# renaudbedard/raytracing-in-one-weekend

Measured on AMD Instinct MI355X. Metric: Msamples/s, 486-sphere cover scene 1920x1080 8-bounce, higher is better.
Workload: dtype f32

## Files before the change

### include/rtow.h

```cpp
#ifndef RTOW_H
#define RTOW_H

#include <stddef.h>
#include <stdint.h>

#ifdef __cplusplus
extern "C" {
#endif

#if defined(_WIN32)
#define RTOW_API __declspec(dllexport)
#else
#define RTOW_API __attribute__((visibility("default")))
#endif

#define RTOW_API_VERSION 12

typedef enum RtowResult {
    RTOW_SUCCESS = 0,
    RTOW_ERROR_INVALID_VALUE = 1,
    RTOW_ERROR_MEMORY_ALLOCATION = 2,
    RTOW_ERROR_NO_DEVICE = 3,
    RTOW_ERROR_NO_SCENE = 4,
    RTOW_ERROR_UNSUPPORTED = 5,
// ... 102 lines not shown
    int32_t sceneInLds;
    uint64_t sceneBytesDevice;
    uint64_t hitSpillBytes;
    int32_t hitListCapacity;
    int32_t wideCodes;
    int32_t thresholdSet;
    int32_t schedulerTune[9];
} RtowSceneInfo;


typedef struct RtowView {
    RtowFloat3 origin;
    RtowFloat3 lowerLeftCorner;
    RtowFloat3 horizontal, vertical;
    RtowFloat3 forward, up, right;
    float lensRadius;
} RtowView;

typedef enum RtowRngPolicy { RTOW_RNG_REFERENCE = 0, RTOW_RNG_PER_SAMPLE = 1, RTOW_RNG_PER_SAMPLE_XOROSHIRO = 2 } RtowRngPolicy;

typedef enum RtowCubemapChannelType { RTOW_CUBEMAP_UNSIGNED_BYTE = 0, RTOW_CUBEMAP_SIGNED_HALF = 1 } RtowCubemapChannelType;
typedef struct RtowCubemapDesc {
    int32_t faceWidth, faceHeight;
    int32_t channelType;
    int32_t pixelStride;
    const void* faces;
} RtowCubemapDesc;

typedef struct RtowBlueNoiseDesc {
    uint32_t rowStride, textureCount;
    const void* texels;
} RtowBlueNoiseDesc;
typedef struct RtowStbNoiseDesc {
    uint32_t rowStride, textureCount;
    const void* scalar;
    const void* vector2;
    const void* cosineUnitVector3;
    const void* unitVector2;
    const void* unitVector3;
} RtowStbNoiseDesc;

typedef struct RtowEnvironment {
    int32_t skyType;
    RtowFloat3 skyBottomColor;
    RtowFloat3 skyTopColor;
} RtowEnvironment;

typedef struct RtowSampleParams {
    RtowFloat2 size;
    int32_t sliceOffset;
    int32_t sliceDivider;
    uint32_t seed;
    RtowView view;
    RtowEnvironment environment;
    uint32_t sampleCountRange[2];
    int32_t traceDepth;
    int32_t subPixelJitter;
    int32_t noiseColor;
    RtowFloat2 sampleCountWeightExtrema;
    int32_t diagnosticsStride;
    int32_t noiseTextureIndex;
    int32_t rngPolicy;
} RtowSampleParams;

typedef struct RtowAccumBuffers {
    float* color;
    float* normal;
    float* albedo;
    float* sampleCountWeight;
} RtowAccumBuffers;

typedef struct RtowContext_t* RtowContext;

typedef void (*RtowLogCallback)(int32_t level, const char* tag, const char* message, void* userData);

typedef enum RtowContextFlags {
    RTOW_CONTEXT_EXACT_TIES_ALWAYS = 1u << 0,
    RTOW_CONTEXT_EXACT_TIES_NEVER = 1u << 1,
    RTOW_CONTEXT_REFERENCE_DIAGNOSTICS = 1u << 2,
    RTOW_CONTEXT_NO_CAMERA_RAY_LISTS = 1u << 3,
    RTOW_CONTEXT_NO_CHUNK_ORDER = 1u << 4,
    RTOW_CONTEXT_FORCE_WIDE_CODES = 1u << 5,
    RTOW_CONTEXT_NO_CHAIN_FUSION = 1u << 7,
    RTOW_CONTEXT_NO_THRESHOLD_TUNING = 1u << 6
} RtowContextFlags;

typedef struct RtowContextOptions {
    int32_t deviceOrdinal;
    RtowLogCallback logCallback;
    void* logCallbackData;
    int32_t logCallbackLevel;
    uint32_t flags;
    int32_t ldsSceneBudgetBytes;
    int32_t schedulerTune[9];
    int32_t hitListCapacity;
    int32_t sliceBlockThreads;
} RtowContextOptions;

RTOW_API int rtowGetApiVersion(void);
RTOW_API const char* rtowErrorString(int result);

RTOW_API int rtowCreateContext(const RtowContextOptions* options, RtowContext* outContext);
RTOW_API int rtowDestroyContext(RtowContext context);

RTOW_API int rtowUploadScene(RtowContext context, const RtowSceneDesc* scene);
RTOW_API int rtowGetSceneInfo(RtowContext context, RtowSceneInfo* outInfo);

RTOW_API int rtowUploadSkyCubemap(RtowContext context, const RtowCubemapDesc* cubemap);

RTOW_API int rtowUploadBlueNoise(RtowContext context, const RtowBlueNoiseDesc* noise);
RTOW_API int rtowUploadStbNoise(RtowContext context, const RtowStbNoiseDesc* noise);

RTOW_API int rtowSampleBatch(RtowContext context, const RtowSampleParams* params,
                             const RtowAccumBuffers* in, const RtowAccumBuffers* out,
                             void* diagnostics, const volatile uint8_t* cancel);

RTOW_API int rtowSampleBatchDevice(RtowContext context, const RtowSampleParams* params,
                                   const RtowAccumBuffers* in, const RtowAccumBuffers* out,
                                   void* diagnostics, void* stream, const volatile uint8_t* cancel);

RTOW_API int rtowSampleBatchChainDevice(RtowContext context, int32_t count, const RtowSampleParams* params ,
                                        const RtowAccumBuffers* in, const RtowAccumBuffers* out,
                                        void* const* diagnostics , void* stream, const volatile uint8_t* cancel);

typedef struct RtowAdaptiveFeed {
    const RtowFloat2* extremaIn;
    RtowFloat2* extremaOut;
    int32_t lag;
    int32_t reserved;
} RtowAdaptiveFeed;

RTOW_API int rtowSampleBatchChainAdaptiveDevice(RtowContext context, int32_t count, const RtowSampleParams* params ,
                                                const RtowAccumBuffers* in, const RtowAccumBuffers* out,
                                                void* const* diagnostics , const RtowAdaptiveFeed* feed,
                                                void* stream, const volatile uint8_t* cancel);

RTOW_API int rtowSampleBatchGroupDevice(RtowContext context, int32_t count, const RtowSampleParams* params ,
                                        const RtowAccumBuffers* in, const RtowAccumBuffers* outs ,
                                        void* const* diagnostics , void* stream, const volatile uint8_t* cancel);

RTOW_API int rtowSampleBatchChain(RtowContext context, int32_t count, const RtowSampleParams* params ,
                                  const RtowAccumBuffers* in, const RtowAccumBuffers* out,
                                  void* const* diagnostics , const volatile uint8_t* cancel);

RTOW_API int rtowRegisterHostBuffer(RtowContext context, void* pointer, size_t sizeInBytes);
RTOW_API int rtowUnregisterHostBuffer(RtowContext context, void* pointer);

RTOW_API int rtowProbeNearestHit(RtowContext context, const RtowFloat3* origin, const RtowFloat3* direction, float time, float* distance, int32_t* entityIndex);

typedef struct RtowRay {
    RtowFloat3 origin;  float time;
    RtowFloat3 direction; float pad;
} RtowRay;

typedef struct RtowHitBuffers {
    float*   distance;
    int32_t* entityIndex;
    float*   normal;
} RtowHitBuffers;

RTOW_API int rtowTraceRaysDevice(RtowContext context, int32_t count, const RtowRay* rays ,
                                 const RtowHitBuffers* hits, void* stream);

typedef struct RtowTraceViewParams {
    int32_t width, height;
    RtowView view;
// ... 161 lines not shown
```

### raytracing-in-one-weekend_amd/abi.py

```python
import ctypes as C

RTOW_API_VERSION = 12

RTOW_SUCCESS = 0
RTOW_ERROR_INVALID_VALUE = 1
RTOW_ERROR_MEMORY_ALLOCATION = 2
RTOW_ERROR_NO_DEVICE = 3
RTOW_ERROR_NO_SCENE = 4
RTOW_ERROR_UNSUPPORTED = 5
RTOW_ERROR_LAUNCH_FAILURE = 6
RTOW_ERROR_CANCELLED = 7
RTOW_ERROR_CAPACITY = 8
RTOW_ERROR_INTERNAL = 99

ENTITY_NONE, ENTITY_SPHERE, ENTITY_RECT, ENTITY_BOX, ENTITY_TRIANGLE = range(5)
MATERIAL_STANDARD, MATERIAL_DIELECTRIC, MATERIAL_PROBABILISTIC_VOLUME = range(3)
TEXTURE_NONE, TEXTURE_CONSTANT, TEXTURE_CHECKER_PATTERN, TEXTURE_PERLIN_NOISE, TEXTURE_IMAGE, TEXTURE_CONSTANT_SCALAR = range(6)
SKY_NONE, SKY_GRADIENT, SKY_CUBEMAP = range(3)
NOISE_WHITE, NOISE_BLUE, NOISE_SPATIOTEMPORAL_BLUE = range(3)
MEMCPY_HOST_TO_HOST, MEMCPY_HOST_TO_DEVICE, MEMCPY_DEVICE_TO_HOST, MEMCPY_DEVICE_TO_DEVICE = range(4)


class Float2(C.Structure):
    _fields_ = [("x", C.c_float), ("y", C.c_float)]
# ... 19 lines not shown


class Image(C.Structure):
    _fields_ = [("width", C.c_int32), ("height", C.c_int32), ("pixelStride", C.c_int32), ("pixels", C.c_void_p)]


class Material(C.Structure):
    _fields_ = [("type", C.c_int32), ("albedo", Texture), ("glossiness", Texture), ("emission", Texture),
                ("metallic", Texture), ("parameter", C.c_float)]


class Entity(C.Structure):
    _fields_ = [("type", C.c_int32), ("moving", C.c_int32), ("rotation", Float4), ("position", Float3),
                ("destinationOffset", Float3), ("timeRange", Float2), ("materialIndex", C.c_int32),
                ("size", Float3), ("contentIndex", C.c_int32)]


class Triangle(C.Structure):
    _fields_ = [("data", Float3 * 3), ("normals", Float3 * 3), ("textureCoordinates", Float2 * 3)]


class SceneDesc(C.Structure):
    _fields_ = [("entities", C.POINTER(Entity)), ("entityCount", C.c_int32),
                ("materials", C.POINTER(Material)), ("materialCount", C.c_int32),
                ("maxBvhDepth", C.c_int32), ("triangles", C.POINTER(Triangle)), ("triangleCount", C.c_int32),
                ("images", C.POINTER(Image)), ("imageCount", C.c_int32)]


class SceneInfo(C.Structure):
    _fields_ = [("entityCount", C.c_int32), ("materialCount", C.c_int32), ("bvhNodeCount", C.c_int32),
                ("bvhDepth", C.c_int32), ("ldsBytesScene", C.c_int32), ("sceneInLds", C.c_int32),
                ("sceneBytesDevice", C.c_uint64), ("hitSpillBytes", C.c_uint64), ("hitListCapacity", C.c_int32), ("wideCodes", C.c_int32),
                ("thresholdSet", C.c_int32), ("schedulerTune", C.c_int32 * 9)]


class View(C.Structure):
    _fields_ = [("origin", Float3), ("lowerLeftCorner", Float3), ("horizontal", Float3), ("vertical", Float3),
                ("forward", Float3), ("up", Float3), ("right", Float3), ("lensRadius", C.c_float)]


CUBEMAP_UNSIGNED_BYTE, CUBEMAP_SIGNED_HALF = 0, 1
RNG_REFERENCE, RNG_PER_SAMPLE, RNG_PER_SAMPLE_XOROSHIRO = 0, 1, 2


class CubemapDesc(C.Structure):
    _fields_ = [("faceWidth", C.c_int32), ("faceHeight", C.c_int32), ("channelType", C.c_int32), ("pixelStride", C.c_int32),
                ("faces", C.c_void_p)]


class BlueNoiseDesc(C.Structure):
    _fields_ = [("rowStride", C.c_uint32), ("textureCount", C.c_uint32), ("texels", C.c_void_p)]


class StbNoiseDesc(C.Structure):
    _fields_ = [("rowStride", C.c_uint32), ("textureCount", C.c_uint32), ("scalar", C.c_void_p), ("vector2", C.c_void_p),
                ("cosineUnitVector3", C.c_void_p), ("unitVector2", C.c_void_p), ("unitVector3", C.c_void_p)]


class Environment(C.Structure):
    _fields_ = [("skyType", C.c_int32), ("skyBottomColor", Float3), ("skyTopColor", Float3)]


class SampleParams(C.Structure):
    _fields_ = [("size", Float2), ("sliceOffset", C.c_int32), ("sliceDivider", C.c_int32), ("seed", C.c_uint32),
                ("view", View), ("environment", Environment), ("sampleCountRange", C.c_uint32 * 2),
                ("traceDepth", C.c_int32), ("subPixelJitter", C.c_int32), ("noiseColor", C.c_int32),
                ("sampleCountWeightExtrema", Float2), ("diagnosticsStride", C.c_int32), ("noiseTextureIndex", C.c_int32),
                ("rngPolicy", C.c_int32)]


class AccumBuffers(C.Structure):
    _fields_ = [("color", C.c_void_p), ("normal", C.c_void_p), ("albedo", C.c_void_p),
                ("sampleCountWeight", C.c_void_p)]


class AdaptiveFeed(C.Structure):
    _fields_ = [("extremaIn", C.c_void_p), ("extremaOut", C.c_void_p), ("lag", C.c_int32), ("reserved", C.c_int32)]


LogCallback = C.CFUNCTYPE(None, C.c_int32, C.c_char_p, C.c_char_p, C.c_void_p)


CONTEXT_EXACT_TIES_ALWAYS, CONTEXT_EXACT_TIES_NEVER, CONTEXT_REFERENCE_DIAGNOSTICS, CONTEXT_NO_CAMERA_RAY_LISTS, CONTEXT_NO_CHUNK_ORDER, CONTEXT_FORCE_WIDE_CODES, CONTEXT_NO_THRESHOLD_TUNING, CONTEXT_NO_CHAIN_FUSION = 1, 2, 4, 8, 16, 32, 64, 128
GATHER_COLOR, GATHER_NORMAL, GATHER_ALBEDO, GATHER_SAMPLE_COUNT_WEIGHT, GATHER_ALL, GATHER_NO_BATCH_WAIT, GATHER_LOOPBACK = 1, 2, 4, 8, 15, 16, 32


class ContextOptions(C.Structure):
    _fields_ = [("deviceOrdinal", C.c_int32), ("logCallback", LogCallback), ("logCallbackData", C.c_void_p),
                ("logCallbackLevel", C.c_int32), ("flags", C.c_uint32), ("ldsSceneBudgetBytes", C.c_int32), ("schedulerTune", C.c_int32 * 9),
                ("hitListCapacity", C.c_int32), ("sliceBlockThreads", C.c_int32)]


class CommId(C.Structure):
    _fields_ = [("bytes", C.c_char * 128)]


class HybridPlan(C.Structure):
    _fields_ = [("tileCount", C.c_int32), ("groupCount", C.c_int32), ("tile", C.c_int32), ("group", C.c_int32),
                ("sliceOffset", C.c_int32), ("sliceDivider", C.c_int32), ("samples", C.c_uint32), ("seed", C.c_uint32)]


class Metrics(C.Structure):
    _fields_ = [("totalRayCount", C.c_int32), ("totalSamples", C.c_int32), ("sampleCountWeightExtrema", Float2),
                ("sampleCountExtrema", C.c_int32 * 2), ("totalRayCount64", C.c_int64), ("totalSamples64", C.c_int64)]


class CombineParams(C.Structure):
    _fields_ = [("width", C.c_int32), ("height", C.c_int32), ("debugMode", C.c_int32), ("ldrAlbedo", C.c_int32)]


RTOW_DENOISE_DEMODULATE_ALBEDO = 1
DENOISE_DEFAULT_ITERATIONS = 5
DENOISE_DEFAULT_NORMAL_SHARPNESS = 4
DENOISE_DEFAULT_COLOR_SIGMA = 0.5
DENOISE_DEFAULT_ALBEDO_SIGMA = 0.5
DENOISE_DEFAULT_FLAGS = RTOW_DENOISE_DEMODULATE_ALBEDO


class DenoiseParams(C.Structure):
    _fields_ = [("width", C.c_int32), ("height", C.c_int32), ("iterations", C.c_int32), ("normalSharpness", C.c_int32),
                ("colorSigma", C.c_float), ("albedoSigma", C.c_float), ("flags", C.c_int32), ("reserved", C.c_int32)]


class Ray(C.Structure):
    _fields_ = [("origin", Float3), ("time", C.c_float), ("direction", Float3), ("pad", C.c_float)]


RAY_DTYPE = [("origin", "<f4", (3,)), ("time", "<f4"), ("direction", "<f4", (3,)), ("pad", "<f4")]


class RayInterval(C.Structure):
    _fields_ = [("tMin", C.c_float), ("tMax", C.c_float)]


RAY_INTERVAL_DTYPE = [("tMin", "<f4"), ("tMax", "<f4")]


class HitBuffers(C.Structure):
    _fields_ = [("distance", C.c_void_p), ("entityIndex", C.c_void_p), ("normal", C.c_void_p)]


class TraceViewParams(C.Structure):
    _fields_ = [("width", C.c_int32), ("height", C.c_int32), ("view", View), ("time", C.c_float), ("reserved", C.c_int32)]


RTOW_REPROJECT_MATCH_ENTITY = 1
REPROJECT_DEFAULT_DEPTH_TOLERANCE = 0.01
REPROJECT_DEFAULT_MAX_HISTORY = 64
REPROJECT_DEFAULT_FLAGS = RTOW_REPROJECT_MATCH_ENTITY


class ReprojectParams(C.Structure):
    _fields_ = [("width", C.c_int32), ("height", C.c_int32), ("previousView", View), ("depthTolerance", C.c_float), ("maxHistory", C.c_int32),
                ("flags", C.c_int32), ("reserved", C.c_int32)]


RTOW_UPSAMPLE_POINT, RTOW_UPSAMPLE_BILINEAR, RTOW_UPSAMPLE_GUIDED = 0, 1, 2
RTOW_UPSAMPLE_MATCH_ENTITY = 1
RTOW_UPSAMPLE_DEMODULATE_ALBEDO = 2
UPSAMPLE_DEFAULT_MODE = RTOW_UPSAMPLE_GUIDED
UPSAMPLE_DEFAULT_NORMAL_SHARPNESS = 0
UPSAMPLE_DEFAULT_DEPTH_TOLERANCE = 0.2
UPSAMPLE_DEFAULT_FLAGS = RTOW_UPSAMPLE_MATCH_ENTITY | RTOW_UPSAMPLE_DEMODULATE_ALBEDO
UPSAMPLE_MAX_SIZE = 16384


# ... 37 lines not shown
```

### raytracing-in-one-weekend_amd/csrc/rtow_api.hip

```cpp
#include <hip/hip_runtime.h>

#include <algorithm>
#include <atomic>
#include <cfloat>
#include <chrono>
#include <cstdio>
#include <cstring>
#include <mutex>
#include <string>
#include <thread>
#include <vector>

#include "../../include/rtow.h"
#include "rtow_context.h"

#ifndef RTOW_GROUP_SLOT_BLOCK
#define RTOW_GROUP_SLOT_BLOCK 4
#endif
static constexpr unsigned kGroupSlotBlock = RTOW_GROUP_SLOT_BLOCK;
#ifndef RTOW_PIXEL_GATE
#define RTOW_PIXEL_GATE 1
#endif
#ifndef RTOW_URGENT_RAYS_PER_SAMPLE
#define RTOW_URGENT_RAYS_PER_SAMPLE 18.0f
// ... 44 lines not shown
}

struct ChainSpec { int count; const uint32_t* seeds; void* const* diags; const RtowAccumBuffers* outs; const RtowFloat2* const* extrema = nullptr; unsigned* extremaKeys = nullptr; };

void dropThresholdTuning(RtowContext ctx)
{
    for (auto& e : ctx->tuneEvents) if (e) (void)hipEventDestroy(e);
    ctx->tuneEvents.clear();
    ctx->tunePending = false;
}

uint64_t sceneSignature(const CompiledScene& sc, bool wide)
{
    return ((uint64_t)sc.layout.sceneKind << 60) ^ ((uint64_t)(sc.layout.exactTies ? 1 : 0) << 59) ^ ((uint64_t)(wide ? 1 : 0) << 58) ^ ((uint64_t)sc.layout.nodeCount << 29) ^
           (uint64_t)(uint32_t)sc.entityCount ^ ((uint64_t)sc.layout.materialCount << 44);
}

bool finishThresholdTuning(RtowContext ctx, bool wait)
{
    if (!ctx->tunePending || ctx->tuneEvents.empty()) return false;
    const hipError_t q = wait ? hipEventSynchronize(ctx->tuneEvents.back()) : hipEventQuery(ctx->tuneEvents.back());
    if (q == hipErrorNotReady) { (void)hipGetLastError(); return false; }
    const int candidates = ctx->tuneCandidates, builtin = ctx->tuneBuiltin;
    bool ok = q == hipSuccess;
    float best = 0.0f, builtinMs = 0.0f;
    int winner = -1;
    for (int c = 0; ok && c < candidates; c++) {
        float t = 0.0f;
        for (int r = 0; r < kTuneProbeRepeats; r++) {
            float ms = 0.0f;
            if (hipEventElapsedTime(&ms, ctx->tuneEvents[(size_t)(r * candidates + c)], ctx->tuneEvents[(size_t)(r * candidates + c) + 1]) != hipSuccess) { ms = 1e30f; (void)hipGetLastError(); }
            t = (r == 0 || ms < t) ? ms : t;
        }
        if (c == builtin) builtinMs = t;
        if (winner < 0 || t < best) { best = t; winner = c; }
    }
    if (ok && winner >= 0) {
        if (winner != builtin && !(best < kTuneMargin * builtinMs)) { winner = builtin; best = builtinMs; }
        candidateThresholds(winner, ctx->tune, 8);
        ctx->tunedCandidate = winner;
        ctx->tuneCache.push_back({ctx->sceneSignatureNow, winner});
        logf(ctx, 4, "tune", "stage thresholds measured on this scene: candidate %d of %d (%.3f ms per %d-sample probe)", winner, candidates, best, kTuneProbeSamples);
    } else {
        (void)hipGetLastError();
        ctx->tunedCandidate = -1;
        logf(ctx, 2, "tune", "threshold probes failed; the per-kind values stay");
    }
    ctx->tunedScene = ctx->tunePendingScene;
    dropThresholdTuning(ctx);
    return true;
}

uint64_t listCapacity(const RtowContext_t* ctx, bool volumes);
inline bool triangleKind(uint32_t kind) { return kind == SCENE_KIND_TRIANGLES || kind == SCENE_KIND_TRIANGLES_TEXTURED; }
constexpr unsigned kTieWatchBusy = 4096;

const char* sampleKernelName(const SceneLayout& L)
{
    const bool ties = L.exactTies != 0;
    switch (L.sceneKind) {
        case SCENE_KIND_SPHERES: return ties ? "sample_spheres_ties" : "sample_spheres";
        case SCENE_KIND_SPHERES_MOTION: return ties ? "sample_spheres_motion_ties" : "sample_spheres_motion";
        case SCENE_KIND_VOLUMES: return "sample_volumes";
        case SCENE_KIND_TEXTURED: return ties ? "sample_textured_ties" : "sample_textured";
        case SCENE_KIND_VOLUMES_TEXTURED: return "sample_volumes_textured";
        case SCENE_KIND_TRIANGLES_TEXTURED: return ties ? "sample_triangles_textured_ties" : "sample_triangles_textured";
        case SCENE_KIND_TRIANGLES: return ties ? "sample_triangles_ties" : "sample_triangles";
        default: return ties ? "sample_general_ties" : "sample_general";
    }
}


int buildArgs(RtowContext ctx, const RtowSampleParams* p, const RtowAccumBuffers* in, const RtowAccumBuffers* out, void* diag, bool useCancelFlag, const ChainSpec* chain,
              const RtowFloat2* extremaIn, SampleKernelArgs& a)
{
    a.inColor = in->color; a.inNormal = in->normal; a.inAlbedo = in->albedo; a.inScw = in->sampleCountWeight;
    a.outColor = out->color; a.outNormal = out->normal; a.outAlbedo = out->albedo; a.outScw = out->sampleCountWeight;
    a.diagnostics = (uint8_t*)diag;
    a.diagnosticsStride = p->diagnosticsStride;
    a.sceneBlob = ctx->dScene;
    a.layout = ctx->scene.layout;
    a.ldsSceneBytes = ctx->ldsSceneBytes;
    a.ldsNodeCount = ctx->ldsNodeCount;
    a.ldsStackRows = ctx->ldsPlan.stackRows; a.ldsHistOffset = 0u; a.ldsFrontBytes = ctx->ldsPlan.frontBytes;
    a.workCounter = ctx->dWorkCounter;
    a.cancelFlag = useCancelFlag ? ctx->hCancel : nullptr;
    a.overflowFlag = const_cast<uint32_t*>(ctx->hCancel) + 1;
    a.width = (int)p->size.x;
    a.height = (int)p->size.y;
    a.totalWork = (uint32_t)ownedRows(p) * (uint32_t)a.width;
    a.tilesPerRow = (RTOW_TICKET_TILES && a.width % (int)kTileW == 0) ? (uint32_t)a.width / kTileW : 0u;
    a.tiledPixels = a.tilesPerRow ? ((uint32_t)ownedRows(p) / kTileH) * kTileH * (uint32_t)a.width : 0u;
    a.sizeX = p->size.x; a.sizeY = p->size.y;
    a.sliceOffset = p->sliceOffset; a.sliceDivider = p->sliceDivider;
    a.seed = chain ? chain->seeds[0] : p->seed;
    a.chainCount = chain ? (uint32_t)chain->count : 1u;
    a.chainIndependent = (chain && chain->outs) ? 1 : 0;
    a.groupRecip = a.chainCount <= 1u ? 0xffffffffu : (uint32_t)((1ull << 32) / a.chainCount + 1ull);
    if (chain) {
        if (diag == nullptr && chain->diags) diag = chain->diags[0];
        a.diagnostics = (uint8_t*)diag;
    }
    a.view = p->view;
    a.environment = p->environment;
    a.sampleCountMin = p->sampleCountRange[0];
    a.sampleCountMax = p->sampleCountRange[1];
    a.traceDepth = p->traceDepth;
    a.subPixelJitter = p->subPixelJitter;
    a.extremaX = p->sampleCountWeightExtrema.x;
    a.extremaY = p->sampleCountWeightExtrema.y;
    a.extremaIn = extremaIn;
    a.refTree = (ctx->flags & RTOW_CONTEXT_REFERENCE_DIAGNOSTICS) ? ctx->dRefTree : nullptr;
    a.hitSpill = ctx->hitSpillEntries ? ctx->dHitSpill : nullptr;
    a.hitSpillEntries = ctx->hitSpillEntries;
    a.hitSpillStride = (uint32_t)ctx->cuCount * (uint32_t)kBlockThreads;
    a.tex.blob = ctx->dTexBlob;
    a.tex.layout = ctx->scene.texLayout;
    a.noiseColor = p->noiseColor;
    if (p->noiseColor == RTOW_NOISE_BLUE) {
        if (!ctx->dBlueNoise || p->noiseTextureIndex < 0 || (uint32_t)p->noiseTextureIndex >= ctx->blueTextureCount) return RTOW_ERROR_INVALID_VALUE;
        a.blueRowStride = ctx->blueRowStride;
        a.blueNoise = ctx->dBlueNoise + (size_t)p->noiseTextureIndex * ctx->blueRowStride * ctx->blueRowStride * 8u;
    } else if (p->noiseColor == RTOW_NOISE_SPATIOTEMPORAL_BLUE) {
        if (!ctx->dStbNoise || p->noiseTextureIndex < 0 || (uint32_t)p->noiseTextureIndex >= ctx->stbTextureCount) return RTOW_ERROR_INVALID_VALUE;
        const size_t texels = (size_t)ctx->stbRowStride * ctx->stbRowStride, all = texels * ctx->stbTextureCount, t = (size_t)p->noiseTextureIndex * texels;
        a.stbRowStride = ctx->stbRowStride;
        a.stbScalar = ctx->dStbNoise + t;
        a.stbVector2 = ctx->dStbNoise + all + t * 3;
        a.stbCosineUnitVector3 = ctx->dStbNoise + all * 4 + t * 4;
        a.stbUnitVector2 = ctx->dStbNoise + all * 8 + t * 3;
        a.stbUnitVector3 = ctx->dStbNoise + all * 11 + t * 3;
    }
    a.cubemap = cubemapRefs(ctx->cubemap, ctx->dCubemap);
    return RTOW_SUCCESS;
}

int planHistory(RtowContext ctx, const RtowSampleParams* p, SampleKernelArgs& a)
{
    const bool fullDiag = a.diagnostics && a.diagnosticsStride >= 16;
    const bool perSample = p->rngPolicy != RTOW_RNG_REFERENCE;
    int hw = historyWords(a.noiseColor, perSample, ctx->wideCodes, ctx->scene.layout.exactTies != 0, fullDiag, a.traceDepth);
    if (ctx->scene.layout.exactTies) hw = std::max(hw, historyWords(a.noiseColor, perSample, ctx->wideCodes, false, fullDiag, a.traceDepth));
    if (hw != 32 || a.traceDepth <= kHistoryInRegisters) return RTOW_SUCCESS;
    const LdsPlan plan = planLds(ctx->wideCodes, ctx->scene.layout, (uint32_t)(a.traceDepth - kHistoryInRegisters), ctx->ldsSceneBudget);
    a.ldsStackRows = plan.stackRows; a.ldsHistOffset = plan.histOffset; a.ldsFrontBytes = plan.frontBytes; a.ldsHistRows = plan.histRows;
    a.ldsSceneBytes = plan.sceneBytes; a.ldsNodeCount = plan.nodeCount;
    if (plan.histSpillRows) {
        const size_t stride = (size_t)ctx->cuCount * (size_t)kBlockThreads, need = (size_t)plan.histSpillRows * stride * sizeof(unsigned short);
        if (need > ctx->histSpillBytes) HIP_TRY(ctx, hipDeviceSynchronize(), RTOW_ERROR_LAUNCH_FAILURE);
        RTOW_TRY(growDevice(ctx, ctx->histSpillBytes, need, {devBuf(ctx->dHistSpill, need)}));
        a.histSpill = ctx->dHistSpill; a.histSpillRows = plan.histSpillRows; a.histSpillStride = (uint32_t)stride;
    }
    return RTOW_SUCCESS;
}

void setSchedulerValues(const RtowContext_t* ctx, const RtowSampleParams* p, SampleKernelArgs& a)
{
    for (int i = 0; i < 8; i++) a.tune[i] = ctx->tune[i] < 1 ? 1 : ctx->tune[i];
    a.travSlice = ctx->tune[8] < 1 ? 1 : ctx->tune[8];
    const unsigned unitSamples = p->rngPolicy != RTOW_RNG_REFERENCE ? kSampleGroup : (a.sampleCountMax > a.sampleCountMin ? a.sampleCountMax : a.sampleCountMin);
    const int pixelGate = ctx->pixelGateOverride ? ctx->pixelGateOverride : (unitSamples <= 64u ? 4 : RTOW_PIXEL_GATE);
    const bool records16 = a.diagnostics && a.diagnosticsStride >= 16;
    const bool twin = !a.chainIndependent && p->rngPolicy == RTOW_RNG_REFERENCE &&
                      hurryTwin(a.layout.sceneKind, a.layout.exactTies != 0, ctx->wideCodes, a.noiseColor, false, records16, a.refTree != nullptr, a.traceDepth);
    const float urgentRays = !twin ? __builtin_inff() : (a.ldsSceneBytes == a.layout.totalBytes ? RTOW_URGENT_RAYS_PER_SAMPLE : RTOW_URGENT_RAYS_PER_SAMPLE_BEYOND_LDS);
    uint32_t bits;
    memcpy(&bits, &urgentRays, sizeof bits);
    if (!(urgentRays < __builtin_inff())) bits = 0u;
    a.tune[7] = (int32_t)((bits & 0xffffff00u) | (uint32_t)(pixelGate & 255));
}

int recordEmptyBatch(RtowContext ctx, hipStream_t stream)
{
    if (ctx->haveBatchDone) HIP_TRY(ctx, hipStreamWaitEvent(stream, ctx->evBatchDone, 0), RTOW_ERROR_LAUNCH_FAILURE);
    HIP_TRY(ctx, hipEventRecord(ctx->evStart, stream), RTOW_ERROR_LAUNCH_FAILURE);
    HIP_TRY(ctx, hipEventRecord(ctx->evStop, stream), RTOW_ERROR_LAUNCH_FAILURE);
    HIP_TRY(ctx, hipEventRecord(ctx->evBatchDone, stream), RTOW_ERROR_LAUNCH_FAILURE);
    ctx->haveBatchDone = true;
    ctx->haveTiming = true;
    return RTOW_SUCCESS;
}

int planUnits(RtowContext ctx, const RtowSampleParams* p, SampleKernelArgs& a)
{
    a.groupsPerPixel = 1;
    a.xoroshiro = p->rngPolicy == RTOW_RNG_PER_SAMPLE_XOROSHIRO ? 1 : 0;
    if (p->rngPolicy == RTOW_RNG_REFERENCE) return RTOW_SUCCESS;
    const uint32_t ownedPixels = a.totalWork;
    uint32_t groups = (a.sampleCountMax > a.sampleCountMin ? a.sampleCountMax : a.sampleCountMin);
    groups = (groups + kSampleGroup - 1) / kSampleGroup;
    if (groups < 1) groups = 1;
    if ((uint64_t)ownedPixels * groups > 0x7fffffffull) return RTOW_ERROR_CAPACITY;
    a.groupsPerPixel = groups;
    a.totalWork = ownedPixels * groups;
    RTOW_TRY(growDevice(ctx, ctx->unitRecordCapacity, a.totalWork, {devBuf(ctx->dUnitRecords, (size_t)a.totalWork * 64u)}));
    a.unitRecords = ctx->dUnitRecords;
    return RTOW_SUCCESS;
}

struct TieWatch {
    bool on = false;
    bool triangles = false;
    bool inPlace = false;
};

int prepareTieWatch(RtowContext ctx, const RtowSampleParams* p, const RtowAccumBuffers* in, const RtowAccumBuffers* out, SampleKernelArgs& a, TieWatch& tie)
{
    if (ctx->hCancel[3] != 0u) { ctx->hCancel[3] = 0u; if (triangleKind(ctx->scene.layout.sceneKind)) { ctx->triWatchOff = true; logf(ctx, 3, "rtow", "this scene's nearest hits tie often: exact-tie kernels from now on"); } }
    const bool sphereWatch = ctx->scene.layout.sceneKind <= SCENE_KIND_SPHERES_MOTION && !ctx->scene.layout.exactTies && ctx->scene.entityCount > 16;
    tie.triangles = triangleKind(ctx->scene.layout.sceneKind) && ctx->scene.layout.exactTies && ctx->scene.layout.tieWatchOk && !ctx->triWatchOff &&
                    !(ctx->flags & RTOW_CONTEXT_EXACT_TIES_ALWAYS);
    tie.on = (sphereWatch || tie.triangles) && !(ctx->flags & RTOW_CONTEXT_EXACT_TIES_NEVER) && p->rngPolicy == RTOW_RNG_REFERENCE;
    if (tie.on && tie.triangles) a.layout.exactTies = 0u;
    tie.inPlace = in->color == out->color || in->normal == out->normal || in->albedo == out->albedo || in->sampleCountWeight == out->sampleCountWeight;
    if (!tie.on) return RTOW_SUCCESS;
    if (!ctx->dTieRedo) HIP_TRY(ctx, hipMalloc(&ctx->dTieRedo, (4u + (size_t)kTieRedoCapacity) * sizeof(unsigned)), RTOW_ERROR_MEMORY_ALLOCATION);
    const uint32_t most = (uint32_t)std::min<uint64_t>((uint64_t)ctx->scene.entityCount, listCapacity(ctx, false));
    const uint32_t entries = most > (uint32_t)kLocalHitEntries ? most - (uint32_t)kLocalHitEntries : 0u;
    RTOW_TRY(growDevice(ctx, ctx->redoSpillEntries, entries, {devBuf(ctx->dRedoSpill, (size_t)entries * kTieRedoBlocks * kBlockThreads * sizeof(uint4))}));
    const size_t framePixels = (size_t)a.width * (size_t)a.height;
    const size_t words = (framePixels + 31u) / 32u;
    RTOW_TRY(growDevice(ctx, ctx->tieBitsWords, words, {devBuf(ctx->dTieBits, words * sizeof(unsigned))}));
    if (tie.inPlace) RTOW_TRY(growDevice(ctx, ctx->tieInputPixels, framePixels, {devBuf(ctx->dTieInputs, framePixels * 11u * sizeof(float))}));
    return RTOW_SUCCESS;
}

int refreshCameraRays(RtowContext ctx, SampleKernelArgs& a, uint32_t ownedPixels, hipStream_t stream)
{
    if (ctx->flags & RTOW_CONTEXT_NO_CAMERA_RAY_LISTS) return RTOW_SUCCESS;
    const size_t pixels = (size_t)a.width * (size_t)a.height;
    const size_t listBytes = pixels * sizeof(uint4);
    if (listBytes > ctx->pixCandCapacity) ctx->pixCandValid = false;
    RTOW_TRY(growDevice(ctx, ctx->pixCandCapacity, listBytes, {devBuf(ctx->dPixCand, listBytes)}));
    const bool same = ctx->pixCandValid && ctx->pixCandScene == ctx->sceneSerial && memcmp(&ctx->pixCandView, &a.view, sizeof(RtowView)) == 0 &&
                      ctx->pixCandW == a.width && ctx->pixCandH == a.height && ctx->pixCandOff == a.sliceOffset && ctx->pixCandDiv == a.sliceDivider &&
                      ctx->pixCandJitter == (a.subPixelJitter ? 1 : 0);
    if (!same) {
        SampleKernelArgs perPixel = a;
        perPixel.totalWork = ownedPixels;
        HIP_TRY(ctx, launchPrimaryCandidates(perPixel, ctx->dPixCand, stream), RTOW_ERROR_LAUNCH_FAILURE);
        ctx->pixCandValid = true;
        ctx->pixCandScene = ctx->sceneSerial;
// ... 641 lines not shown
    if (ctx->dColor) { (void)hipFree(ctx->dColor); (void)hipFree(ctx->dNormal); (void)hipFree(ctx->dAlbedo); (void)hipFree(ctx->dScw); }
    if (ctx->dDiag) (void)hipFree(ctx->dDiag);
    releaseComm(ctx);
    for (const RtowContext_t::HostRange& r : ctx->hostRanges) (void)hipHostUnregister(r.base);
    ctx->hostRanges.clear();
    if (ctx->evStart) (void)hipEventDestroy(ctx->evStart);
    if (ctx->evStop) (void)hipEventDestroy(ctx->evStop);
    if (ctx->evBatchDone) (void)hipEventDestroy(ctx->evBatchDone);
    if (ctx->evMetricsDone) (void)hipEventDestroy(ctx->evMetricsDone);
    if (ctx->stream) (void)hipStreamDestroy(ctx->stream);
    delete ctx;
    return RTOW_SUCCESS;
}

RTOW_API int rtowUploadScene(RtowContext ctx, const RtowSceneDesc* scene)
{
    if (!ctx || !scene) return RTOW_ERROR_INVALID_VALUE;
    std::lock_guard<std::mutex> lock(ctx->mu);
    HIP_TRY(ctx, hipSetDevice(ctx->device), RTOW_ERROR_NO_DEVICE);
    CompiledScene compiled;
    std::string err;
    const int rc = compileScene(scene, RTOW_STACK_CAPACITY, &compiled, &err);
    if (rc != RTOW_SUCCESS) {
        logf(ctx, 2, "scene", "%s", err.c_str());
        return rc;
    }
    HIP_TRY(ctx, hipDeviceSynchronize(), RTOW_ERROR_LAUNCH_FAILURE);
    RTOW_TRY(growDevice(ctx, ctx->dSceneCapacity, compiled.blob.size(), {devBuf(ctx->dScene, compiled.blob.size())}));
    HIP_TRY(ctx, hipMemcpy(ctx->dScene, compiled.blob.data(), compiled.blob.size(), hipMemcpyHostToDevice), RTOW_ERROR_LAUNCH_FAILURE);
    if (!compiled.entityOfPrim.empty()) {
        const size_t n = compiled.entityOfPrim.size();
        RTOW_TRY(growDevice(ctx, ctx->entityOfPrimCapacity, n, {devBuf(ctx->dEntityOfPrim, n * sizeof(int32_t))}));
        HIP_TRY(ctx, hipMemcpy(ctx->dEntityOfPrim, compiled.entityOfPrim.data(), n * sizeof(int32_t), hipMemcpyHostToDevice), RTOW_ERROR_LAUNCH_FAILURE);
    }
    if (ctx->dPrimOfEntity) { (void)hipFree(ctx->dPrimOfEntity); ctx->dPrimOfEntity = nullptr; }
    ctx->primOfEntityCount = 0;
    if (!compiled.entityOfPrim.empty() && compiled.entityCount > 0) {
        std::vector<int32_t> primOfEntity((size_t)compiled.entityCount, -1);
        for (size_t prim = 0; prim < compiled.entityOfPrim.size(); prim++) {
            const int32_t entity = compiled.entityOfPrim[prim];
            if (entity >= 0 && entity < compiled.entityCount) primOfEntity[(size_t)entity] = (int32_t)prim;
        }
        HIP_TRY(ctx, hipMalloc((void**)&ctx->dPrimOfEntity, primOfEntity.size() * sizeof(int32_t)), RTOW_ERROR_MEMORY_ALLOCATION);
        HIP_TRY(ctx, hipMemcpy(ctx->dPrimOfEntity, primOfEntity.data(), primOfEntity.size() * sizeof(int32_t), hipMemcpyHostToDevice), RTOW_ERROR_LAUNCH_FAILURE);
        ctx->primOfEntityCount = compiled.entityCount;
    }
    if (!compiled.texBlob.empty()) {
        RTOW_TRY(growDevice(ctx, ctx->texBlobCapacity, compiled.texBlob.size(), {devBuf(ctx->dTexBlob, compiled.texBlob.size())}));
        HIP_TRY(ctx, hipMemcpy(ctx->dTexBlob, compiled.texBlob.data(), compiled.texBlob.size(), hipMemcpyHostToDevice), RTOW_ERROR_LAUNCH_FAILURE);
        compiled.texBlob.clear();
        compiled.texBlob.shrink_to_fit();
    }
    if (ctx->flags & RTOW_CONTEXT_REFERENCE_DIAGNOSTICS) {
        if (compiled.refTreeDepth > 62) { logf(ctx, 2, "scene", "RTOW_CONTEXT_REFERENCE_DIAGNOSTICS supports MaxBvhDepth <= 62"); return RTOW_ERROR_CAPACITY; }
        RTOW_TRY(growDevice(ctx, ctx->refTreeCapacity, compiled.refTree.size(), {devBuf(ctx->dRefTree, compiled.refTree.size())}));
        HIP_TRY(ctx, hipMemcpy(ctx->dRefTree, compiled.refTree.data(), compiled.refTree.size(), hipMemcpyHostToDevice), RTOW_ERROR_LAUNCH_FAILURE);
    }
    compiled.refTree.clear();
    compiled.refTree.shrink_to_fit();
    HIP_TRY(ctx, launchPrepareMaterials(ctx->dScene, compiled.layout, ctx->stream), RTOW_ERROR_LAUNCH_FAILURE);
    HIP_TRY(ctx, launchPrepareEntities(ctx->dScene, compiled.layout, ctx->stream), RTOW_ERROR_LAUNCH_FAILURE);
    HIP_TRY(ctx, hipStreamSynchronize(ctx->stream), RTOW_ERROR_LAUNCH_FAILURE);
    if (compiled.layout.sceneKind >= SCENE_KIND_GENERAL && compiled.entityCount > 0)
        HIP_TRY(ctx, hipMemcpy(compiled.blob.data() + compiled.layout.primOffset, ctx->dScene + compiled.layout.primOffset, (size_t)compiled.entityCount * sizeof(GpuPrim), hipMemcpyDeviceToHost),
                RTOW_ERROR_LAUNCH_FAILURE);
    if (ctx->flags & (RTOW_CONTEXT_EXACT_TIES_ALWAYS | RTOW_CONTEXT_EXACT_TIES_NEVER)) {
        const bool volumes = compiled.layout.sceneKind == SCENE_KIND_VOLUMES || compiled.layout.sceneKind == SCENE_KIND_VOLUMES_TEXTURED;
        if (!volumes) compiled.layout.exactTies = (ctx->flags & RTOW_CONTEXT_EXACT_TIES_ALWAYS) ? 1u : 0u;
    }
    {
        const int rc = sizeHitSpill(ctx, compiled.layout.sceneKind, compiled.layout.exactTies != 0, compiled.entityCount);
        if (rc != RTOW_SUCCESS) return rc;
    }
    const bool wide = compiled.entityCount > 65535 || compiled.layout.nodeCount > 65535u || (ctx->flags & RTOW_CONTEXT_FORCE_WIDE_CODES) != 0;
    ctx->wideCodes = wide;
    if (!ctx->userTune) {
        const int* base = kThresholdFamilies[compiled.layout.sceneKind <= SCENE_KIND_SPHERES_MOTION ? 0 : 1];
        for (int k = 0; k < 9; k++) ctx->tune[k] = base[k];
    } else if (ctx->userSliceDefault) {
        ctx->tune[8] = 16;
    }
    std::lock_guard<std::mutex> sceneLock(ctx->sceneMu);
    ctx->scene = std::move(compiled);
    ctx->ldsPlan = planLds(wide, ctx->scene.layout, 0u, ctx->ldsSceneBudget);
    ctx->ldsSceneBytes = ctx->ldsPlan.sceneBytes;
    ctx->ldsNodeCount = ctx->ldsPlan.nodeCount;
    ctx->haveScene = true;
    ctx->triWatchOff = false;
    ctx->hCancel[3] = 0u;
    ctx->sceneSerial++;
    ctx->orderValid = false;
    dropThresholdTuning(ctx);
    ctx->sppSinceUpload = 0;
    ctx->sceneSignatureNow = sceneSignature(ctx->scene, wide);
    if (!ctx->userTune && !(ctx->flags & RTOW_CONTEXT_NO_THRESHOLD_TUNING))
        for (const RtowContext_t::TuneCacheEntry& e : ctx->tuneCache)
            if (e.signature == ctx->sceneSignatureNow) {
                candidateThresholds(e.winner, ctx->tune, 8);
                ctx->tunedCandidate = e.winner;
                ctx->tunedScene = ctx->sceneSerial;
            }
    logf(ctx, 4, "scene", "%d entities, %u BVH nodes, depth %u, %u bytes (%u in LDS)%s", ctx->scene.entityCount, ctx->scene.layout.nodeCount,
         ctx->scene.layout.bvhDepth, ctx->scene.layout.totalBytes, ctx->ldsSceneBytes,
         ctx->scene.layout.exactTies ? ", exact-tie kernels" : "");
    return RTOW_SUCCESS;
}

RTOW_API int rtowUploadSkyCubemap(RtowContext ctx, const RtowCubemapDesc* cubemap)
{
    if (!ctx) return RTOW_ERROR_INVALID_VALUE;
    std::lock_guard<std::mutex> lock(ctx->mu);
    HIP_TRY(ctx, hipSetDevice(ctx->device), RTOW_ERROR_NO_DEVICE);
    if (!cubemap || !cubemap->faces) {
        HIP_TRY(ctx, hipDeviceSynchronize(), RTOW_ERROR_LAUNCH_FAILURE);
        if (ctx->dCubemap) (void)hipFree(ctx->dCubemap);
        ctx->dCubemap = nullptr;
        ctx->cubemapCapacity = 0;
        ctx->cubemap = RtowCubemapDesc{};
        return RTOW_SUCCESS;
    }
    if (cubemap->faceWidth <= 0 || cubemap->faceHeight <= 0 || cubemap->faceWidth > 32768 || cubemap->faceHeight > 32768) return RTOW_ERROR_INVALID_VALUE;
    if (cubemap->channelType != RTOW_CUBEMAP_UNSIGNED_BYTE && cubemap->channelType != RTOW_CUBEMAP_SIGNED_HALF) return RTOW_ERROR_INVALID_VALUE;
    const int minStride = cubemap->channelType == RTOW_CUBEMAP_SIGNED_HALF ? 6 : 3;
    if (cubemap->pixelStride < minStride || cubemap->pixelStride > 64) return RTOW_ERROR_INVALID_VALUE;
    if (cubemap->channelType == RTOW_CUBEMAP_SIGNED_HALF && (cubemap->pixelStride & 1)) return RTOW_ERROR_INVALID_VALUE;
    const size_t bytes = (size_t)6 * (size_t)cubemap->faceWidth * (size_t)cubemap->faceHeight * (size_t)cubemap->pixelStride;
    if (bytes > 0x7fffffffull) return RTOW_ERROR_CAPACITY;
    HIP_TRY(ctx, hipDeviceSynchronize(), RTOW_ERROR_LAUNCH_FAILURE);
    if (bytes > ctx->cubemapCapacity) ctx->cubemap = RtowCubemapDesc{};
    RTOW_TRY(growDevice(ctx, ctx->cubemapCapacity, bytes, {devBuf(ctx->dCubemap, bytes)}));
    HIP_TRY(ctx, hipMemcpy(ctx->dCubemap, cubemap->faces, bytes, hipMemcpyHostToDevice), RTOW_ERROR_LAUNCH_FAILURE);
    ctx->cubemap = *cubemap;
    ctx->cubemap.faces = nullptr;
    logf(ctx, 3, "sky", "cubemap %dx%d, %s, stride %d (%zu bytes)", cubemap->faceWidth, cubemap->faceHeight,
         cubemap->channelType == RTOW_CUBEMAP_SIGNED_HALF ? "half" : "byte", cubemap->pixelStride, bytes);
    return RTOW_SUCCESS;
}

RTOW_API int rtowUploadBlueNoise(RtowContext ctx, const RtowBlueNoiseDesc* noise)
{
    if (!ctx) return RTOW_ERROR_INVALID_VALUE;
    std::lock_guard<std::mutex> lock(ctx->mu);
    HIP_TRY(ctx, hipSetDevice(ctx->device), RTOW_ERROR_NO_DEVICE);
    HIP_TRY(ctx, hipDeviceSynchronize(), RTOW_ERROR_LAUNCH_FAILURE);
    if (ctx->dBlueNoise) (void)hipFree(ctx->dBlueNoise);
    ctx->dBlueNoise = nullptr;
    ctx->blueRowStride = ctx->blueTextureCount = 0;
    if (!noise || !noise->texels) return RTOW_SUCCESS;
    if (noise->rowStride == 0 || noise->rowStride > 16384 || noise->textureCount == 0 || noise->textureCount > 4096) return RTOW_ERROR_INVALID_VALUE;
    const size_t bytes = (size_t)noise->rowStride * noise->rowStride * noise->textureCount * 8u;
    HIP_TRY(ctx, hipMalloc(&ctx->dBlueNoise, bytes), RTOW_ERROR_MEMORY_ALLOCATION);
    HIP_TRY(ctx, hipMemcpy(ctx->dBlueNoise, noise->texels, bytes, hipMemcpyHostToDevice), RTOW_ERROR_LAUNCH_FAILURE);
    ctx->blueRowStride = noise->rowStride;
    ctx->blueTextureCount = noise->textureCount;
    return RTOW_SUCCESS;
}

RTOW_API int rtowUploadStbNoise(RtowContext ctx, const RtowStbNoiseDesc* noise)
{
    if (!ctx) return RTOW_ERROR_INVALID_VALUE;
    std::lock_guard<std::mutex> lock(ctx->mu);
    HIP_TRY(ctx, hipSetDevice(ctx->device), RTOW_ERROR_NO_DEVICE);
    HIP_TRY(ctx, hipDeviceSynchronize(), RTOW_ERROR_LAUNCH_FAILURE);
    if (ctx->dStbNoise) (void)hipFree(ctx->dStbNoise);
    ctx->dStbNoise = nullptr;
    ctx->stbRowStride = ctx->stbTextureCount = 0;
    if (!noise) return RTOW_SUCCESS;
    if (!noise->scalar || !noise->vector2 || !noise->cosineUnitVector3 || !noise->unitVector2 || !noise->unitVector3) return RTOW_ERROR_INVALID_VALUE;
    if (noise->rowStride == 0 || noise->rowStride > 16384 || noise->textureCount == 0 || noise->textureCount > 4096) return RTOW_ERROR_INVALID_VALUE;
    const size_t all = (size_t)noise->rowStride * noise->rowStride * noise->textureCount;
    HIP_TRY(ctx, hipMalloc(&ctx->dStbNoise, all * 14u), RTOW_ERROR_MEMORY_ALLOCATION);
    HIP_TRY(ctx, hipMemcpy(ctx->dStbNoise, noise->scalar, all, hipMemcpyHostToDevice), RTOW_ERROR_LAUNCH_FAILURE);
    HIP_TRY(ctx, hipMemcpy(ctx->dStbNoise + all, noise->vector2, all * 3, hipMemcpyHostToDevice), RTOW_ERROR_LAUNCH_FAILURE);
    HIP_TRY(ctx, hipMemcpy(ctx->dStbNoise + all * 4, noise->cosineUnitVector3, all * 4, hipMemcpyHostToDevice), RTOW_ERROR_LAUNCH_FAILURE);
    HIP_TRY(ctx, hipMemcpy(ctx->dStbNoise + all * 8, noise->unitVector2, all * 3, hipMemcpyHostToDevice), RTOW_ERROR_LAUNCH_FAILURE);
    HIP_TRY(ctx, hipMemcpy(ctx->dStbNoise + all * 11, noise->unitVector3, all * 3, hipMemcpyHostToDevice), RTOW_ERROR_LAUNCH_FAILURE);
    ctx->stbRowStride = noise->rowStride;
    ctx->stbTextureCount = noise->textureCount;
    return RTOW_SUCCESS;
}

RTOW_API int rtowGetSceneInfo(RtowContext ctx, RtowSceneInfo* info)
{
    if (!ctx || !info) return RTOW_ERROR_INVALID_VALUE;
    std::lock_guard<std::mutex> lock(ctx->mu);
    if (!ctx->haveScene) return RTOW_ERROR_NO_SCENE;
    if (ctx->tunePending && hipSetDevice(ctx->device) == hipSuccess) (void)finishThresholdTuning(ctx,  false);
    info->entityCount = ctx->scene.entityCount;
    info->materialCount = ctx->scene.materialCount;
    info->bvhNodeCount = (int32_t)ctx->scene.layout.nodeCount;
    info->bvhDepth = (int32_t)ctx->scene.layout.bvhDepth;
    info->ldsBytesScene = (int32_t)ctx->ldsSceneBytes;
    info->sceneInLds = ctx->ldsSceneBytes == ctx->scene.layout.totalBytes ? 1 : 0;
    info->sceneBytesDevice = ctx->scene.layout.totalBytes;
    info->hitSpillBytes = (uint64_t)ctx->hitSpillEntries * (uint64_t)ctx->cuCount * (uint64_t)kBlockThreads * sizeof(uint4);
    const bool keepsLists = ctx->scene.layout.exactTies || ctx->scene.layout.sceneKind == SCENE_KIND_VOLUMES || ctx->scene.layout.sceneKind == SCENE_KIND_VOLUMES_TEXTURED;
    const bool tieWatch = ctx->scene.layout.sceneKind <= SCENE_KIND_SPHERES_MOTION && !ctx->scene.layout.exactTies && ctx->scene.entityCount > 16 && !(ctx->flags & RTOW_CONTEXT_EXACT_TIES_NEVER);
    info->hitListCapacity = keepsLists ? (int32_t)(ctx->hitSpillEntries + (uint32_t)kLocalHitEntries)
                                       : tieWatch ? (int32_t)std::min<uint64_t>((uint64_t)ctx->scene.entityCount, listCapacity(ctx, false)) : 0;
    info->wideCodes = ctx->wideCodes ? 1 : 0;
    info->thresholdSet = ctx->tunedScene == ctx->sceneSerial ? ctx->tunedCandidate : -1;
    for (int k = 0; k < 9; k++) info->schedulerTune[k] = ctx->tune[k];
    info->schedulerTune[7] = ctx->schedulerKnob;
    return RTOW_SUCCESS;
}

RTOW_API int rtowSampleBatchDevice(RtowContext ctx, const RtowSampleParams* params, const RtowAccumBuffers* in, const RtowAccumBuffers* out,
                                   void* diagnostics, void* stream, const volatile uint8_t* cancel)
{
    if (!out) return RTOW_ERROR_INVALID_VALUE;
    std::unique_lock<std::mutex> lock;
    hipStream_t s;
    RTOW_TRY(beginSample(ctx, lock, 1, params, in, out, noBatchCheck, stream, &s));
    return enqueueBatches(ctx, 1, params, in, out, &diagnostics, false, false, s, cancel);
}

RTOW_API int rtowSampleBatchChainDevice(RtowContext ctx, int32_t count, const RtowSampleParams* params, const RtowAccumBuffers* in, const RtowAccumBuffers* out,
                                        void* const* diagnostics, void* stream, const volatile uint8_t* cancel)
{
    if (!out) return RTOW_ERROR_INVALID_VALUE;
    std::unique_lock<std::mutex> lock;
    hipStream_t s;
    RTOW_TRY(beginSample(ctx, lock, count, params, in, out, noBatchCheck, stream, &s));
    return enqueueBatches(ctx, count, params, in, out, diagnostics, false, canFuse(ctx, count, params, diagnostics,  true, false), s, cancel);
}

RTOW_API int rtowSampleBatchChainAdaptiveDevice(RtowContext ctx, int32_t count, const RtowSampleParams* params, const RtowAccumBuffers* in, const RtowAccumBuffers* out,
                                                void* const* diagnostics, const RtowAdaptiveFeed* feed, void* stream, const volatile uint8_t* cancel)
{
    if (!out || !feed || feed->lag < 1 || !feed->extremaOut || feed->reserved != 0) return RTOW_ERROR_INVALID_VALUE;
    auto oneFrame = [&](int b) -> int {
        return memcmp(&params[b].size, &params[0].size, sizeof(RtowFloat2)) != 0 || params[b].sliceOffset != params[0].sliceOffset ||
                       params[b].sliceDivider != params[0].sliceDivider || params[b].diagnosticsStride != params[0].diagnosticsStride
                   ? RTOW_ERROR_INVALID_VALUE : RTOW_SUCCESS;
    };
    std::unique_lock<std::mutex> lock;
    hipStream_t s;
    RTOW_TRY(beginSample(ctx, lock, count, params, in, out, oneFrame, stream, &s));
    if (!ctx->dExtremaPartials) HIP_TRY(ctx, hipMalloc(&ctx->dExtremaPartials, sizeof(RtowFloat2) * kMetricsBlocks), RTOW_ERROR_MEMORY_ALLOCATION);
    const int pixels = (int)params[0].size.x * (int)params[0].size.y;
    const int lag = feed->lag;
    auto source = [&](int k) -> const RtowFloat2* { return k < lag ? (feed->extremaIn ? feed->extremaIn + k : nullptr) : feed->extremaOut + (k - lag); };
    const bool fusable = lag > 1 && canFuse(ctx, count, params, diagnostics,  true,  true);
    if (fusable && !ctx->dExtremaKeys) HIP_TRY(ctx, hipMalloc(&ctx->dExtremaKeys, 2u * sizeof(unsigned) * kMaxChain), RTOW_ERROR_MEMORY_ALLOCATION);
    for (int first = 0; first < count;) {
        int n = fusable ? std::min(count - first, std::min(lag, (int)kMaxChain)) : 1;
        for (int b = 1; b < n; b++)
            if (!source(first + b) && memcmp(&params[first + b].sampleCountWeightExtrema, &params[first].sampleCountWeightExtrema, sizeof(RtowFloat2)) != 0) n = 1;
        const RtowAccumBuffers* src = first == 0 ? in : out;
        int rc;
        if (n == 1) {
            rc = launchSample(ctx, &params[first], src, out, diagnostics ? diagnostics[first] : nullptr, s, cancel != nullptr, nullptr, source(first));
            if (rc != RTOW_SUCCESS) return rc;
            HIP_TRY(ctx, launchReduceWeightExtrema(pixels, out->color, out->sampleCountWeight, ctx->dExtremaPartials, feed->extremaOut + first, s), RTOW_ERROR_LAUNCH_FAILURE);
        } else {
            uint32_t seeds[kMaxChain];
            const RtowFloat2* sources[kMaxChain];
            for (int b = 0; b < n; b++) { seeds[b] = params[first + b].seed; sources[b] = source(first + b); }
            if (ctx->haveBatchDone) HIP_TRY(ctx, hipStreamWaitEvent(s, ctx->evBatchDone, 0), RTOW_ERROR_LAUNCH_FAILURE);
            HIP_TRY(ctx, launchInitExtremaKeys(ctx->dExtremaKeys, (unsigned)n, (int)params[0].size.x, (int)params[0].size.y, params[0].sliceOffset, params[0].sliceDivider,
                                               out->color, out->sampleCountWeight, s), RTOW_ERROR_LAUNCH_FAILURE);
            ChainSpec chain{n, seeds, diagnostics ? diagnostics + first : nullptr, nullptr};
            chain.extrema = sources;
            chain.extremaKeys = ctx->dExtremaKeys;
            rc = launchSample(ctx, &params[first], src, out, nullptr, s, cancel != nullptr, &chain);
            if (rc != RTOW_SUCCESS) return rc;
            HIP_TRY(ctx, launchDecodeExtremaKeys(ctx->dExtremaKeys, (unsigned)n, feed->extremaOut + first, s), RTOW_ERROR_LAUNCH_FAILURE);
        }
        HIP_TRY(ctx, hipEventRecord(ctx->evBatchDone, s), RTOW_ERROR_LAUNCH_FAILURE);
        if (cancel) {
            rc = waitWithCancel(ctx, cancel);
            if (rc != RTOW_SUCCESS) return rc;
        }
        first += n;
    }
// ... 463 lines not shown
```

### raytracing-in-one-weekend_amd/csrc/rtow_kernels.h

```cpp
#pragma once
#include <hip/hip_runtime.h>
#include <stdint.h>

#include "../../include/rtow.h"
#include "rtow_bvh.h"
#include "rtow_scene.h"

namespace rtow {

#ifndef RTOW_BLOCK_THREADS
#define RTOW_BLOCK_THREADS 1024
#endif
constexpr int kBlockThreads = RTOW_BLOCK_THREADS;
constexpr int kLdsBytesMax = 160 * 1024;
#ifndef RTOW_TRAV_SLICE
#define RTOW_TRAV_SLICE 8
#endif
constexpr int kCandCapacity = 8;
constexpr int kQueueBytes = 384;
constexpr int kHistoryInRegisters = 8;

struct LdsPlan {
    uint32_t stackRows;
    uint32_t histOffset;
    uint32_t histRows;
    uint32_t histSpillRows;
    uint32_t frontBytes;
    uint32_t sceneBytes;
    uint32_t nodeCount;
    bool allLds;
};
inline LdsPlan planLds(bool wide, const SceneLayout& L, uint32_t histRowsNeeded, uint32_t budgetOverride)
{
    LdsPlan p{};
    const uint32_t codeBytes = wide ? 4u : 2u, rowBytes = (uint32_t)kBlockThreads * 2u;
    p.stackRows = L.bvhDepth < 1u ? 1u : L.bvhDepth;
    const uint32_t rowsEnd = ((uint32_t)kCandCapacity + p.stackRows) * (uint32_t)kBlockThreads * codeBytes + (wide ? 256u : 0u);
    const uint32_t room = (uint32_t)kLdsBytesMax - rowsEnd - (uint32_t)kQueueBytes;
    uint32_t sceneBudget = room;
    if (budgetOverride >= sizeof(GpuNode) && budgetOverride < sceneBudget) sceneBudget = budgetOverride;
    const bool whole = !wide && L.totalBytes <= sceneBudget && (uint64_t)L.totalBytes + (uint64_t)histRowsNeeded * rowBytes <= (uint64_t)room;
    const uint32_t keep = whole ? L.totalBytes : (uint32_t)sizeof(GpuNode) * (L.nodeCount < 256u ? (L.nodeCount ? L.nodeCount : 1u) : 256u);
    const uint32_t keepFits = keep <= sceneBudget ? keep : sceneBudget;
    uint32_t rowsFit = room > keepFits ? (room - keepFits) / rowBytes : 0u;
    p.histRows = histRowsNeeded < rowsFit ? histRowsNeeded : rowsFit;
    p.histSpillRows = histRowsNeeded - p.histRows;
    p.histOffset = p.histRows ? rowsEnd : 0u;
    p.frontBytes = rowsEnd + p.histRows * rowBytes;
    uint32_t budget = (uint32_t)kLdsBytesMax - p.frontBytes - (uint32_t)kQueueBytes;
    if (budget > sceneBudget) budget = sceneBudget;
    if (whole) {
        p.sceneBytes = L.totalBytes; p.nodeCount = L.nodeCount; p.allLds = true;
    } else {
        uint32_t nodes = budget / (uint32_t)sizeof(GpuNode);
        if (nodes > L.nodeCount) nodes = L.nodeCount;
        p.nodeCount = nodes; p.sceneBytes = nodes * (uint32_t)sizeof(GpuNode); p.allLds = false;
    }
    return p;
}
inline int historyWords(int noiseColor, bool perSample, bool wide, bool ties, bool fullDiag, int traceDepth)
{
    if (noiseColor != RTOW_NOISE_WHITE) return 32;
    if (perSample) return (!ties && !wide && !fullDiag && traceDepth <= 8) ? 4 : 32;
    if (fullDiag) return 32;
    if (traceDepth <= 8) return 4;
    if (traceDepth <= 16 && (!wide || ties)) return 8;
    return 32;
}
constexpr unsigned kNoPrimaryList = 0x0000ffffu;
#ifndef RTOW_URGENT_LANES
#define RTOW_URGENT_LANES 1
#endif
inline bool hurryTwin(uint32_t sceneKind, bool ties, bool wide, int noiseColor, bool perSample, bool records16, bool refTree, int traceDepth)
{
    return RTOW_URGENT_LANES && sceneKind == SCENE_KIND_SPHERES && !ties && !wide && noiseColor == RTOW_NOISE_WHITE && !perSample && !(records16 && refTree) &&
           historyWords(noiseColor, perSample, wide, ties, records16, traceDepth) == 32;
}
#ifndef RTOW_SAMPLE_GROUP
#define RTOW_SAMPLE_GROUP 16
#endif
constexpr unsigned kSampleGroup = RTOW_SAMPLE_GROUP;
constexpr unsigned kChunkOrderScratchWords = 1056;
constexpr int kMaxChain = 16;
constexpr int kLocalHitEntries = 24;
constexpr uint32_t kDefaultHitListCapacity = 1024;
constexpr uint32_t kTieRedoCapacity = 1u << 20;
constexpr int kTieRedoBlocks = 8;
constexpr uint32_t kDefaultTieListCapacity = 128;

constexpr unsigned kMaxXcds = 16;
struct XcdState {
    unsigned owned[kMaxXcds];
    unsigned ticket[kMaxXcds];
    unsigned listed;
    unsigned pad[15];
};

struct ChainBatch {
    uint8_t* diagnostics;
    uint32_t seed;
    uint32_t pad;
    float *outColor, *outNormal, *outAlbedo, *outScw;
    const RtowFloat2* extrema;
};

__host__ __device__ inline unsigned extrema_key(float f) { unsigned u; __builtin_memcpy(&u, &f, 4); return (u & 0x80000000u) ? ~u : (u | 0x80000000u); }
__host__ __device__ inline float extrema_value(unsigned k) { const unsigned u = (k & 0x80000000u) ? (k & 0x7fffffffu) : ~k; float f; __builtin_memcpy(&f, &u, 4); return f; }
constexpr unsigned kExtremaMinStart = 0xff800000u;
constexpr unsigned kExtremaMaxStart = 0x007fffffu;

#ifndef RTOW_TICKET_TILES
#define RTOW_TICKET_TILES 1
#endif
#ifndef RTOW_TICKET_TILE_W
#define RTOW_TICKET_TILE_W 8
#endif
constexpr unsigned kTileW = RTOW_TICKET_TILE_W, kTileH = 64u / kTileW;
static_assert(kTileW * kTileH == 64u && (kTileW & (kTileW - 1u)) == 0u, "a tile is one 64-ticket chunk");
__host__ __device__ inline void owned_pixel_xy(unsigned n, unsigned width, unsigned tilesPerRow, unsigned tiledPixels, int& cx, int& ownedRow)
{
    if (n < tiledPixels) {
        const unsigned tile = n >> 6, i = n & 63u;
        const unsigned ty = tile / tilesPerRow, tx = tile - ty * tilesPerRow;
        cx = (int)(tx * kTileW + (i & (kTileW - 1u)));
        ownedRow = (int)(ty * kTileH + i / kTileW);
    } else {
        ownedRow = (int)(n / width);
        cx = (int)(n - (unsigned)ownedRow * width);
    }
}

struct TexRefs {
    const uint8_t* blob;
    TexLayout layout;
};
// ... 19 lines not shown
    const float* inColor;
    const float* inNormal;
    const float* inAlbedo;
    const float* inScw;
    float* outColor;
    float* outNormal;
    float* outAlbedo;
    float* outScw;
    uint8_t* diagnostics;
    int32_t diagnosticsStride;

    const uint8_t* sceneBlob;
    SceneLayout layout;
    uint32_t ldsSceneBytes;
    uint32_t ldsNodeCount;
    uint32_t ldsStackRows, ldsHistOffset, ldsFrontBytes;
    uint32_t ldsHistRows, histSpillRows, histSpillStride;
    unsigned short* histSpill;

    unsigned int* workCounter;
    const unsigned int* chunkOrder;
    unsigned short* pixelCost;
    const unsigned int* ticketMap;
    uint32_t chunkCount;
    uint32_t slotBlock, groupRecip;
    const uint2* pixelCandidates;
    int32_t probeOnly;
    const volatile uint32_t* cancelFlag;
    uint32_t* overflowFlag;
    uint32_t totalWork;
    int32_t width, height;
    uint32_t tilesPerRow, tiledPixels;

    float sizeX, sizeY;
    int32_t sliceOffset, sliceDivider;
    uint32_t seed;
    RtowView view;
    RtowEnvironment environment;
    uint32_t sampleCountMin, sampleCountMax;
    int32_t traceDepth;
    int32_t subPixelJitter;
    float extremaX, extremaY;
    unsigned* extremaKeys;
    const RtowFloat2* extremaIn;

    float* unitRecords;
    uint32_t groupsPerPixel;
    int32_t xoroshiro;

    TexRefs tex;

    int32_t noiseColor;
    uint32_t blueRowStride, stbRowStride;
    const void* blueNoise;
    const uint8_t* stbScalar;
    const uint8_t* stbVector2;
    const uint8_t* stbCosineUnitVector3;
    const uint8_t* stbUnitVector2;
    const uint8_t* stbUnitVector3;

    CubemapRefs cubemap;

    const uint8_t* refTree;

    uint4* hitSpill;
    uint32_t hitSpillEntries, hitSpillStride;

    uint32_t chainCount;
    int32_t chainIndependent;
    const ChainBatch* chainBatches;
    unsigned int* chunkDone;
    XcdState* xcdState;

    unsigned* tieBits;
    unsigned* tieRedo;
    uint32_t tieRedoCapacity;
    int32_t redoMode;

    int32_t blockThreads;
    int32_t wideCodes;

    int32_t tune[8];
    int32_t travSlice;
};

struct KernelInfo {
    int numRegs;
    int sharedSizeBytes;
    int maxDynamicLds;
};

hipError_t launchSampleSpheres(const SampleKernelArgs& args, int numBlocks, hipStream_t stream, bool allLds);
hipError_t launchSampleSpheresMotion(const SampleKernelArgs& args, int numBlocks, hipStream_t stream, bool allLds);
hipError_t launchSampleGeneral(const SampleKernelArgs& args, int numBlocks, hipStream_t stream, bool allLds);
hipError_t launchSampleGeneralTies(const SampleKernelArgs& args, int numBlocks, hipStream_t stream, bool allLds);
hipError_t launchSampleTexturedTies(const SampleKernelArgs& args, int numBlocks, hipStream_t stream, bool allLds);
hipError_t launchSampleSpheresTies(const SampleKernelArgs& args, int numBlocks, hipStream_t stream, bool allLds);
hipError_t launchSampleSpheresMotionTies(const SampleKernelArgs& args, int numBlocks, hipStream_t stream, bool allLds);
hipError_t launchSampleVolumes(const SampleKernelArgs& args, int numBlocks, hipStream_t stream, bool allLds);
hipError_t launchSampleTextured(const SampleKernelArgs& args, int numBlocks, hipStream_t stream, bool allLds);
hipError_t launchSampleVolumesTextured(const SampleKernelArgs& args, int numBlocks, hipStream_t stream, bool allLds);
hipError_t launchSampleTriangles(const SampleKernelArgs& args, int numBlocks, hipStream_t stream, bool allLds);
hipError_t launchSampleTrianglesTies(const SampleKernelArgs& args, int numBlocks, hipStream_t stream, bool allLds);
hipError_t launchSampleTrianglesTextured(const SampleKernelArgs& args, int numBlocks, hipStream_t stream, bool allLds);
hipError_t launchSampleTrianglesTexturedTies(const SampleKernelArgs& args, int numBlocks, hipStream_t stream, bool allLds);
hipError_t launchSampleBatch(const SampleKernelArgs& args, int numBlocks, hipStream_t stream);
hipError_t launchPrepareMaterials(uint8_t* blob, const SceneLayout& layout, hipStream_t stream);
hipError_t launchPrimaryCandidates(const SampleKernelArgs& args, uint2* out, hipStream_t stream);
hipError_t launchFoldUnitRecords(const SampleKernelArgs& args, hipStream_t stream);
hipError_t launchBuildChunkOrder(const unsigned short* pixelCost, unsigned* cost, unsigned chunkCount, unsigned* order, int byMax, hipStream_t stream);
hipError_t launchInitTicketMap(unsigned* ticketMap, unsigned count, hipStream_t stream);
constexpr unsigned kRegroupMaxSide = 8;
hipError_t launchRegroupTickets(unsigned short* pixelCost, unsigned* ticketMap, unsigned tilesPerRow, unsigned tileRows, unsigned side, const unsigned classes[3], hipStream_t stream);
hipError_t launchPrepareEntities(uint8_t* blob, const SceneLayout& layout, hipStream_t stream);
hipError_t launchCombine(const RtowCombineParams& p, const float* inColor, const float* inNormal, const float* inAlbedo,
                         float* outColor, float* outNormal, float* outAlbedo, hipStream_t stream);
constexpr size_t kByteThresholdTableBytes = 259 * sizeof(float);
hipError_t launchBuildByteThresholds(float* thresholds, hipStream_t stream);
hipError_t launchFinalize(int pixelCount, const float* inColor, const float* inNormal, const float* inAlbedo,
                          uint8_t* outColor, uint8_t* outNormal, uint8_t* outAlbedo, const float* thresholds, hipStream_t stream);

hipError_t launchCombineFinalize(const RtowCombineParams& p, const float* inColor, const float* inNormal, const float* inAlbedo,
                                 uint8_t* outColor, uint8_t* outNormal, uint8_t* outAlbedo, const float* thresholds, hipStream_t stream);

hipError_t launchDenoise(const RtowDenoiseParams& p, const float* inColor, const float* inNormal, const float* inAlbedo, float* scratch, float* outColor,
                         hipStream_t stream);
struct ReprojectConstants { float LF, LR, LU, HR, VU; };
inline ReprojectConstants reprojectConstants(const RtowView& v)
{
    const auto dot = [](const RtowFloat3& a, const RtowFloat3& b) { return (a.x * b.x + a.y * b.y) + a.z * b.z; };
    return ReprojectConstants{dot(v.lowerLeftCorner, v.forward), dot(v.lowerLeftCorner, v.right), dot(v.lowerLeftCorner, v.up), dot(v.horizontal, v.right), dot(v.vertical, v.up)};
}
hipError_t launchReproject(const RtowReprojectParams& p, const ReprojectConstants& k, const RtowRay* rays, const RtowHitBuffers& hits, const RtowHitBuffers& previousHits,
                           const RtowAccumBuffers& previous, const RtowAccumBuffers& out, int32_t* outSource, hipStream_t stream);
hipError_t launchUpsample(const RtowUpsampleParams& p, const float* srcColor, const RtowHitBuffers& srcHits, const float* srcAlbedo, const RtowHitBuffers& dstHits,
                          const float* dstAlbedo, float* outColor, uint8_t* outStage, hipStream_t stream);
hipError_t launchAddAccum(size_t pixels, float* const dst[4], const float* const src[4], hipStream_t stream);
hipError_t launchCollectTiedPixels(const unsigned* tieBits, unsigned words, unsigned* tieRedo, unsigned capacity, unsigned batches, uint32_t* overflowFlag, unsigned busyAt, hipStream_t stream);

bool probeNearestHitHost(const uint8_t* blob, const SceneLayout& L, const int32_t* entityOfPrim, const float origin[3], const float direction[3], float time, float* distance, int* entity);

bool probeIntervalHost(const uint8_t* blob, const SceneLayout& L, const int32_t* entityOfPrim, const float origin[3], const float direction[3], float time, float tMin, float tMax,
                       bool any, float* distance, int* entity);

hipError_t launchTraceRays(const uint8_t* blob, const SceneLayout& layout, const int32_t* entityOfPrim, int64_t count, const RtowRay* rays, const RtowHitBuffers& hits,
                           hipStream_t stream);
hipError_t launchTraceView(const uint8_t* blob, const SceneLayout& layout, const int32_t* entityOfPrim, const RtowTraceViewParams& p, const RtowHitBuffers& hits,
                           RtowRay* outRays, hipStream_t stream);

hipError_t launchTraceRaysInterval(const uint8_t* blob, const SceneLayout& layout, const int32_t* entityOfPrim, int64_t count, const RtowRay* rays,
                                   const RtowRayInterval* intervals, const RtowHitBuffers& hits, hipStream_t stream);
hipError_t launchTraceOcclusion(const uint8_t* blob, const SceneLayout& layout, int64_t count, const RtowRay* rays, const RtowRayInterval* intervals, uint8_t* occluded,
                                hipStream_t stream);

struct ShadeScene {
    const uint8_t* blob;
    SceneLayout layout;
    const int32_t* primOfEntity;
    int32_t entityCount;
    const uint8_t* texBlob;
    TexLayout texLayout;
    const uint8_t* cubemapData;
    RtowCubemapDesc cubemap;
};
hipError_t launchShadeHits(const ShadeScene& scene, const RtowEnvironment& environment, int32_t count, const RtowRay* rays, const int32_t* entityIndex,
                           const RtowSurfaceBuffers& surface, hipStream_t stream);
// ... 17 lines not shown
```

### raytracing-in-one-weekend_amd/csrc/rtow_sample_kernel.hip.h

```cpp
#pragma once
#include "rtow_kernels.h"

#include <type_traits>

#include "rtow_detmath.hip.h"
#include "rtow_hit_tests.hip.h"
#include "rtow_surface.hip.h"
#include "rtow_vecmath.hip.h"

#ifndef RTOW_WHOLE_MATERIAL
#define RTOW_WHOLE_MATERIAL 1
#endif
#ifndef RTOW_LDS_VIEW
#define RTOW_LDS_VIEW 2
#endif
#ifndef RTOW_COLD_VIEW
#define RTOW_COLD_VIEW 1
#endif
#ifndef RTOW_TRI_HOT
#define RTOW_TRI_HOT 1
#endif
#ifndef RTOW_PREFETCH
#define RTOW_PREFETCH 0
#endif
#ifndef RTOW_PINHOLE
#define RTOW_PINHOLE 1
#endif
#ifndef RTOW_TIE_WATCH
#define RTOW_TIE_WATCH 1
#endif

namespace rtow {

namespace {

__device__ __forceinline__ float inv_pow2(int depth)
{
    if (depth <= 126) return __uint_as_float((unsigned)(127 - depth) << 23);
    if (depth == 127) return __uint_as_float(0x00400000u);
    return 0.0f;
}

__device__ __forceinline__ float rng_next(unsigned& state)
{
    const unsigned t = state;
    unsigned s = t;
    s ^= s << 13;
    s ^= s >> 17;
    s ^= s << 5;
    state = s;
    return __uint_as_float(0x3f800000u | (t >> 9)) - 1.0f;
}

__device__ __forceinline__ V3 tangent_to_world(float tx, float ty, float tz, V3 n)
{
    const float s = n.z >= 0 ? 1.0f : -1.0f;
    const float a = -RTOW_RCP(s + n.z);
    const float b = n.x * n.y * a;
    const V3 tangent = v3(1 + s * n.x * n.x * a, s * b, -s * n.x);
    const V3 bitangent = v3(b, s + n.y * n.y * a, -n.y);
    const V3 r = v3(tangent.x * tx + n.x * ty + bitangent.x * tz,
                    tangent.y * tx + n.y * ty + bitangent.y * tz,
                    tangent.z * tx + n.z * ty + bitangent.z * tz);
    return normalize(r);
}
__device__ __forceinline__ V3 cosine_hemisphere_uv(float u, float v, V3 n)
{
    const float radius = RTOW_SQRT(u);
    const float theta = v * 2 * kPi;
    float sinT, cosT;
    det_sincos(theta, sinT, cosT);
    const float tx = radius * cosT, tz = radius * sinT;
    const float ty = RTOW_SQRT(1 - u);
    return tangent_to_world(tx, ty, tz, n);
}
__device__ __forceinline__ V3 direction_uv(float r0, float r1)
{
    const float z = r0 * 2.0f - 1.0f;
    const float rr = RTOW_SQRT(um_max(1.0f - z * z, 0.0f));
    const float angle = r1 * kPi * 2.0f;
    float sn, cs;
    det_sincos(angle, sn, cs);
    return v3(cs * rr, sn * rr, z);
}

struct NoiseSite { const SampleKernelArgs* A; unsigned cx, cy; };

__device__ __forceinline__ unsigned noise_texel(unsigned n, unsigned rowStride, unsigned cx, unsigned cy)
{
    constexpr float g = 1.32471795724474602596f;
    constexpr float a1 = 1.0f / g;
    constexpr float a2 = 1.0f / (g * g);
    const float fn = (float)(n - 1u);
    const float x = 0.5f + a1 * fn, y = 0.5f + a2 * fn;
    const float rx = x - __builtin_floorf(x), ry = y - __builtin_floorf(y);
    const unsigned ox = (unsigned)__builtin_floorf(rx * (float)rowStride), oy = (unsigned)__builtin_floorf(ry * (float)rowStride);
    return ((cy + oy) % rowStride) * rowStride + ((cx + ox) % rowStride);
}

template <int NOISE>
struct Rng;

template <>
struct Rng<RTOW_NOISE_WHITE> {
    unsigned s;
    __device__ __forceinline__ void begin_pixel(const NoiseSite&, unsigned pix, unsigned seed)
    {
        s = (seed * 0x8C4CA03Fu) ^ (pix * 0x7383ED49u);
        (void)rng_next(s);
// ... 437 lines not shown
                                                                       uint32_t* overflowFlag, HitSpill spill)
{
    const SceneLayout& L = *layoutInKernarg;
    float hitT[kLocalHits], hitDummy[kLocalHits];
    unsigned hitCode[kLocalHits];
    int n = 0;
    V3 inv = v3(RTOW_RCP(rd.x), RTOW_RCP(rd.y), RTOW_RCP(rd.z));
    if (inv.x != inv.x) inv.x = __builtin_inff();
    if (inv.y != inv.y) inv.y = __builtin_inff();
    if (inv.z != inv.z) inv.z = __builtin_inff();
    const bool twoChildren = L.sphereCount > 1u;
    const float a = dot(rd, rd);
    int sp = 0, cur = 0;
    while (cur >= 0) {
        float4 q0, q1, q2;
        int c0, c1;
        load_node<ALL_LDS>(sc, L, cur, q0, q1, q2, c0, c1);
        const float t0x = (q0.x - ro.x) * inv.x, t1x = (q1.z - ro.x) * inv.x, u0x = (q0.y - ro.x) * inv.x, u1x = (q1.w - ro.x) * inv.x;
        const float t0y = (q0.z - ro.y) * inv.y, t1y = (q2.x - ro.y) * inv.y, u0y = (q0.w - ro.y) * inv.y, u1y = (q2.y - ro.y) * inv.y;
        const float t0z = (q1.x - ro.z) * inv.z, t1z = (q2.z - ro.z) * inv.z, u0z = (q1.y - ro.z) * inv.z, u1z = (q2.w - ro.z) * inv.z;
        const float tmin0 = vmax3(vmin(t0x, t1x), vmin(t0y, t1y), vmax(vmin(t0z, t1z), 0.0f)), tfar0 = vmin3(vmax(t0x, t1x), vmax(t0y, t1y), vmax(t0z, t1z));
        const float tmin1 = vmax3(vmin(u0x, u1x), vmin(u0y, u1y), vmax(vmin(u0z, u1z), 0.0f)), tfar1 = vmin3(vmax(u0x, u1x), vmax(u0y, u1y), vmax(u0z, u1z));
        const bool hit0 = tmin0 <= tfar0, hit1 = tmin1 <= tfar1 && twoChildren;
        for (int side = 0; side < 2; side++) {
            const int cc = side ? c1 : c0;
            if (cc >= 0 || !(side ? (hit1 && tmin1 < tfar1) : (hit0 && tmin0 < tfar0))) continue;
            const int i = ~cc;
            float t;
            bool ok;
            if (KIND >= SCENE_KIND_GENERAL) {
                constexpr bool TRI = KIND == SCENE_KIND_TRIANGLES || KIND == SCENE_KIND_TRIANGLES_TEXTURED;
                const unsigned type = TRI ? (unsigned)RTOW_ENTITY_TRIANGLE : *reinterpret_cast<const unsigned*>(section<ALL_LDS>(sc, L.matIndexOffset) + (uint32_t)i * 4u) >> kPrimTypeShift;
                V3 nl; float4 rq;
                if (TRI && RTOW_TRI_HOT) { float uu, vv; ok = tri_hit_hot<ALL_LDS>(sc, L, i, ro, rd, 0.0f, t, uu, vv); }
                else ok = general_hit<ALL_LDS, TRI>(sc, L, i, type, ro, rd, rtime, 0.0f, t, nl, rq);
            } else {
                V3 c; float r;
                sphere_at<ALL_LDS, KIND == SCENE_KIND_SPHERES_MOTION>(sc, L, i, rtime, c, r);
                ok = sphere_hit(sub(ro, c), rd, a, r, t);
            }
            if (!ok) continue;
            if ((unsigned)n < (unsigned)kLocalHits + spill.entries) { hit_set(hitT, hitDummy, hitCode, spill, n, HitRec{t, 0.0f, (unsigned)i}); n++; }
            else *overflowFlag = 1u;
        }
        const bool in0 = hit0 && c0 >= 0, in1 = hit1 && c1 >= 0;
        if (in0 && in1) { stack[sp * BT] = (Code)c1; sp++; cur = c0; }
        else if (in0 || in1) cur = in0 ? c0 : c1;
        else if (sp > 0) { sp--; cur = (int)stack[sp * BT]; }
        else cur = -1;
    }
    if (n == 0) return -1;
    const unsigned* rank = reinterpret_cast<const unsigned*>(section<ALL_LDS>(sc, L.rankOffset));
    if (n > kLocalHits) sort_hit_list_spilled(hitT, hitDummy, hitCode, spill, n, rank);
    else if (n > 1) sort_hit_list(hitT, hitDummy, hitCode, n, rank);
    return (int)(hitCode[0] & kHitPrimMask);
}

__device__ __noinline__ __attribute__((unused)) float2 reference_counts(const uint8_t* tree, V3 ro, V3 rd)
{
    V3 inv = v3(RTOW_RCP(rd.x), RTOW_RCP(rd.y), RTOW_RCP(rd.z));
    if (inv.x != inv.x) inv.x = __builtin_inff();
    if (inv.y != inv.y) inv.y = __builtin_inff();
    if (inv.z != inv.z) inv.z = __builtin_inff();
    int stack[64];
    int sp = 0;
    stack[sp++] = 0;
    float bh = 0, cc = 0;
    while (sp > 0) {
        const int node = stack[--sp];
        const float4 a = reinterpret_cast<const float4*>(tree)[2 * node], b = reinterpret_cast<const float4*>(tree)[2 * node + 1];
        const float t0x = (a.x - ro.x) * inv.x, t0y = (a.y - ro.y) * inv.y, t0z = (a.z - ro.z) * inv.z;
        const float t1x = (b.x - ro.x) * inv.x, t1y = (b.y - ro.y) * inv.y, t1z = (b.z - ro.z) * inv.z;
        const float tMin = um_max(0.0f, um_max(um_max(um_min(t0x, t1x), um_min(t0y, t1y)), um_min(t0z, t1z)));
        const float tMax = um_min(um_min(um_max(t0x, t1x), um_max(t0y, t1y)), um_max(t0z, t1z));
        if (!(tMin < tMax)) continue;
        bh += 1.0f;
        const int left = __float_as_int(a.w);
        if (left < 0) cc += (float)(~left);
        else if (sp <= 62) { stack[sp++] = left; stack[sp++] = __float_as_int(b.w); }
    }
    return make_float2(bh, cc);
}

constexpr int kGeoWide = 4;
constexpr int kGeoPinhole = 8;
constexpr int kGeoHurry = 16;
constexpr int geo_block_threads(int) { return kBlockThreads; }

template <bool ALL_LDS, int KIND, int HW, int DIAG, int NOISE, bool PER_SAMPLE, int GEO = 0>
__global__ void __launch_bounds__(geo_block_threads(GEO)) sample_batch_kernel(const SampleKernelArgs A)
{
    constexpr bool FULL_DIAG = DIAG != 0;
    extern __shared__ __attribute__((aligned(16))) uint8_t smem[];
    const int tid = (int)threadIdx.x;
    constexpr int BT = geo_block_threads(GEO);
    if (A.redoMode) { if (__hip_atomic_load(A.tieRedo, __ATOMIC_RELAXED, __HIP_MEMORY_SCOPE_AGENT) == 0u) return; }
    constexpr bool WIDE = (GEO & kGeoWide) != 0;
    constexpr bool PINHOLE = (GEO & kGeoPinhole) != 0;
    constexpr bool LONG_LISTS = !WIDE && (KIND & 7) <= SCENE_KIND_SPHERES_MOTION;
    constexpr bool LDS_VIEW = (RTOW_LDS_VIEW & (ALL_LDS ? 1 : 2)) != 0;
    constexpr bool COLD_VIEW __attribute__((unused)) = RTOW_COLD_VIEW && !ALL_LDS && !LDS_VIEW;
    constexpr bool SPLIT_NODES = !ALL_LDS && !WIDE;
    using Code = typename std::conditional<WIDE, unsigned, unsigned short>::type;
    const uint32_t ldsFront = A.ldsFrontBytes;

    const int swizzled = (tid & ~63) + ((tid & 31) << 1) + ((tid >> 5) & 1);
    Code* const cand = reinterpret_cast<Code*>(smem) + (WIDE ? tid : swizzled);
    Code* const stack = cand + kCandCapacity * BT;
    HistRowsT<!ALL_LDS> histRows;
    histRows.lane = HW == 32 ? reinterpret_cast<unsigned short*>(smem + A.ldsHistOffset) + swizzled : nullptr;
    volatile unsigned* const waveQueue = reinterpret_cast<volatile unsigned*>(smem + ldsFront) + (tid >> 6) * 4;
    uint8_t* const ldsScene = smem + ldsFront + kQueueBytes;
    if ((tid & 63) == 0) { waveQueue[0] = 0; waveQueue[1] = 0; waveQueue[2] = 0; waveQueue[3] = 0; }
    float* const ldsConst = reinterpret_cast<float*>(smem + ldsFront + 256);
#if defined(__HIP_DEVICE_COMPILE__)
    if (LDS_VIEW && tid < 31) {
        const uint8_t* const ka = (const uint8_t*)__builtin_amdgcn_kernarg_segment_ptr();
        const size_t from = tid < 22 ? __builtin_offsetof(SampleKernelArgs, view) + 4u * (size_t)tid
                          : tid < 29 ? __builtin_offsetof(SampleKernelArgs, environment) + 4u * (size_t)(tid - 22)
                                     : __builtin_offsetof(SampleKernelArgs, sizeX) + 4u * (size_t)(tid - 29);
        ldsConst[tid] = *reinterpret_cast<const float*>(ka + from);
    }
#endif
    {
        const uint4* src = reinterpret_cast<const uint4*>(A.sceneBlob);
        uint4* dst = reinterpret_cast<uint4*>(ldsScene);
        const uint32_t n16 = A.ldsSceneBytes >> 4;
        for (uint32_t i = (uint32_t)tid; i < n16; i += BT) dst[i] = src[i];
    }
    __syncthreads();

    SceneRefs sc;
    sc.lds = ldsScene;
    sc.glob = A.sceneBlob;
    sc.ldsNodeCount = A.ldsNodeCount;
    const SceneLayout L = A.layout;
    const int traceDepth = A.traceDepth;
    const bool refDiag = DIAG == 2 && A.refTree != nullptr;
    const bool chained = A.chainCount > 1u;
    const bool twoChildren = L.sphereCount > 1u;
    constexpr int BASE = KIND & 7;
    constexpr bool EXACT_TIES = (KIND & kExactTiesBit) != 0;
    constexpr bool HAS_MOTION = BASE == SCENE_KIND_SPHERES_MOTION;
    constexpr bool GENERAL = BASE >= SCENE_KIND_GENERAL;
    constexpr bool VOLUMES = BASE == SCENE_KIND_VOLUMES || BASE == SCENE_KIND_VOLUMES_TEXTURED;
    constexpr bool TEXTURED = BASE == SCENE_KIND_TEXTURED || BASE == SCENE_KIND_VOLUMES_TEXTURED || BASE == SCENE_KIND_TRIANGLES_TEXTURED;
    constexpr bool TRI_KIND = BASE == SCENE_KIND_TRIANGLES || BASE == SCENE_KIND_TRIANGLES_TEXTURED;
    constexpr bool TIE_WATCH = RTOW_TIE_WATCH && (!GENERAL || TRI_KIND) && !EXACT_TIES && !PER_SAMPLE;
    constexpr bool REDO_CAPABLE = (!GENERAL || TRI_KIND) && EXACT_TIES && !PER_SAMPLE;

    int st = ST_REGEN;
    int pix = -1;
    unsigned tick = 0;
    typename std::conditional<PER_SAMPLE && NOISE == RTOW_NOISE_WHITE, RngPerSample, Rng<NOISE>>::type rng{};
    V3 fbNormal = v3(0, 0, 0), fbAlbedo = v3(0, 0, 0);
    unsigned unitGroup = 0;
    unsigned smp = 0, nsamp = 0;
    int cx = 0, cy = 0;
    V3 colorAcc = v3(0, 0, 0), normalAcc = v3(0, 0, 0), albedoAcc = v3(0, 0, 0);
    float scwAcc = 0, scw0 = 0;
    int sampleCount = 0;
    float rayCount = 0, boundsHits = 0, candidates = 0;

    V3 ro = v3(0, 0, 0), rd = v3(0, 0, 1);
    float rtime = 0;
    int depth = 0;
    Hist<HW> hist;
    hist.clear();
    V3 sampleNormal = v3(0, 0, 0);
    int firstNs = -1;
    float randomEventsLocal = 0;

    float texHist[TEXTURED ? HW * 2 * 6 : 1];
    constexpr int kMaxHits = VOLUMES ? kLocalHits : 1;
    float hitT[kMaxHits], hitTmin0[kMaxHits];
    unsigned hitCode[kMaxHits];
    bool tieAtBest = false;
    bool hitOverflow = false;
    int nHits = 0;
    int curVol = -1;
    float pendRE = 0;
    bool insideHit = false;
    float hitTmin = 0;
    constexpr bool TRIANGLES_ONLY = BASE == SCENE_KIND_TRIANGLES || BASE == SCENE_KIND_TRIANGLES_TEXTURED;
    constexpr bool TRI_HOT = TRIANGLES_ONLY && RTOW_TRI_HOT;
    constexpr bool PREFETCH_FAR = WIDE && !ALL_LDS && (RTOW_PREFETCH & 1) != 0;
    constexpr bool PREFETCH_TRI = WIDE && !ALL_LDS && TRI_HOT && (RTOW_PREFETCH & 2) != 0;
    const uint32_t ldsDump __attribute__((unused)) = (uint32_t)(uintptr_t)(__attribute__((address_space(3))) uint8_t*)(smem + ((uint32_t)kCandCapacity + A.ldsStackRows) * (uint32_t)BT * 4u);
    constexpr bool KEEP_NORMAL = BASE == SCENE_KIND_GENERAL || BASE == SCENE_KIND_TRIANGLES;
    V3 keptNormal = v3(0, 0, 0);

    V3 inv = v3(0, 0, 0);
    int cur = 0, sp = 0, nc = 0, prim = -1;
    float best = 0;

    auto endSample = [&](bool ok, V3 sampleColor, V3 skyColor) {
        V3 sampleAlbedo = ok ? skyColor : v3(0, 0, 0);
        if (firstNs >= 0) {
            const unsigned code = hist.get(firstNs, histRows);
            const bool white = (code & 0x8000u) != 0;
            if (TEXTURED) {
                const V3 refl = white ? v3(1, 1, 1) : v3(texHist[firstNs * 6 + 0], texHist[firstNs * 6 + 1], texHist[firstNs * 6 + 2]);
                sampleAlbedo = add(v3(texHist[firstNs * 6 + 3], texHist[firstNs * 6 + 4], texHist[firstNs * 6 + 5]), refl);
            } else {
                const uint8_t* mp = section<ALL_LDS>(sc, L.materialOffset) + (code & 0x7fffu) * 64u;
                const float4 m0 = *reinterpret_cast<const float4*>(mp);
                const float2 m1 = *reinterpret_cast<const float2*>(mp + 16);
                const V3 refl = white ? v3(1, 1, 1) : v3(m0.x, m0.y, m0.z);
                sampleAlbedo = add(v3(m0.w, m1.x, m1.y), refl);
            }
        }
        if (ok) {
            scwAcc += randomEventsLocal;
            colorAcc = add(colorAcc, sampleColor);
            normalAcc = add(normalAcc, sampleNormal);
            albedoAcc = add(albedoAcc, sampleAlbedo);
            sampleCount++;
        } else if (PER_SAMPLE) {
            if (smp == 0) { fbNormal = sampleNormal; fbAlbedo = sampleAlbedo; }
        } else if (smp == 0 && sampleCount == 0 && !A.probeOnly) {
            const SampleKernelArgs& R = A;
            float* fbN = R.outNormal;
            float* fbA = R.outAlbedo;
            if (chained && R.chainIndependent) { fbN = R.chainBatches[tick >> kChainShift].outNormal; fbA = R.chainBatches[tick >> kChainShift].outAlbedo; }
            fbN += 3 * (size_t)pix;
            fbA += 3 * (size_t)pix;
            fbN[0] = sampleNormal.x; fbN[1] = sampleNormal.y; fbN[2] = sampleNormal.z;
            fbA[0] = sampleAlbedo.x; fbA[1] = sampleAlbedo.y; fbA[2] = sampleAlbedo.z;
        }
        smp++;
        st = ST_REGEN;
    };
    auto startRay = [&]() {
        inv = v3(RTOW_RCP_NAN_TO_INF(rd.x), RTOW_RCP_NAN_TO_INF(rd.y), RTOW_RCP_NAN_TO_INF(rd.z));
        cur = 0; sp = 0; nc = 0; prim = -1;
        best = __builtin_inff();
        tieAtBest = false;
        nHits = 0;
        st = ST_TRAV;
        if (DIAG == 2) { if (refDiag) { const float2 rc = reference_counts(A.refTree, ro, rd); boundsHits += rc.x; candidates += rc.y; } }
    };
    auto classify = [&]() {
        rayCount += 1.0f;
        if (VOLUMES) { st = ST_VOL; return; }
        st = prim < 0 ? ST_SKY : ST_HIT;
    };

    uint4 pcand = make_uint4(WIDE ? 0xffffffffu : kNoPrimaryList, 0u, 0u, 0u);
    int force = -1;
    constexpr bool HURRY = RTOW_URGENT_LANES && (GEO & kGeoHurry) != 0;
    unsigned trip = 0;
    STAT_DECL;
    STAGE_DECL;
    for (;;) {
        STAT_ADD(0, 1);
        STAGE_MARK_TOP(7);
        if (chained) { trip++; if ((trip & 7u) == 0u && st == ST_IDLE) st = ST_REGEN; }
        const unsigned long long liveMask = __ballot(st != ST_DEAD && st != ST_IDLE);
        const int live = (int)__popcll(liveMask);
        auto need = [&](int sixtyFourths) { const int t = (live * sixtyFourths + 63) >> 6; return t < 1 ? 1 : t; };
        constexpr unsigned kHurryGrace = 2u;
        unsigned long long hurry = 0ull;
        if (HURRY) hurry = liveMask & __ballot(rayCount > __int_as_float(A.tune[7] & ~255) * (float)(smp + kHurryGrace));
        auto due = [&](bool waiting, int stage, int sixtyFourths) {
            const unsigned long long m = __ballot(waiting);
            return (int)__popcll(m) >= (force == stage ? 1 : need(sixtyFourths)) || (HURRY && (m & hurry) != 0ull);
        };
        bool ran = false;
        constexpr bool PIXEL_COMPANY = HW == 32 || PER_SAMPLE;
        bool regenReady = st == ST_REGEN;
        const int pixelGate = HURRY ? A.tune[7] & 255 : A.tune[7];
        if (PIXEL_COMPANY && pixelGate > 1) {
            const int wantPixel = (int)__popcll(__ballot(st == ST_REGEN && smp >= nsamp));
            const int company = live < pixelGate ? live : pixelGate;
            if (wantPixel < company && force != ST_REGEN) regenReady = st == ST_REGEN && (smp < nsamp || (HURRY && ((hurry >> (tid & 63)) & 1ull) != 0ull));
        }
        if (due(regenReady, ST_REGEN, A.tune[0])) {
            ran = true;
            STAGE_MARK(0);
            STAT_ADD(1, 1);
            if (regenReady) {
                STAT_LANES(2);
                while (smp >= nsamp) {
#if defined(__HIP_DEVICE_COMPILE__)
                    const SampleKernelArgs* coldArgs = (const SampleKernelArgs*)__builtin_amdgcn_kernarg_segment_ptr();
                    asm volatile("" : "+s"(coldArgs));
#else
                    const SampleKernelArgs* coldArgs = &A;
#endif
                    const SampleKernelArgs& C = *coldArgs;
                    const bool grouped = chained && C.chainIndependent != 0;
                    const bool redo = REDO_CAPABLE && C.redoMode != 0;
                    const unsigned tk = chained ? (tick & kChainTicketMask) : tick;
                    const unsigned batch = chained ? (tick >> kChainShift) : 0u;
                    if (pix >= 0 && C.pixelCost) {
                        const unsigned rc = (unsigned)rayCount;
                        C.pixelCost[tk] = (unsigned short)(rc < 65535u ? rc : 65535u);
                    }
                    if (VOLUMES && hitOverflow) { *C.overflowFlag = 1u; hitOverflow = false; }
                    if (pix >= 0 && C.probeOnly) pix = -1;
                    bool redoContinue = false;
                    if (PER_SAMPLE && pix >= 0) {
                        const bool fallback = unitGroup == 0 && sampleCount == 0;
                        float4* rec = reinterpret_cast<float4*>(C.unitRecords) + (size_t)tick * 4u;
                        rec[0] = make_float4(colorAcc.x, colorAcc.y, colorAcc.z, (float)sampleCount);
                        rec[1] = fallback ? make_float4(fbNormal.x, fbNormal.y, fbNormal.z, rayCount) : make_float4(normalAcc.x, normalAcc.y, normalAcc.z, rayCount);
                        rec[2] = fallback ? make_float4(fbAlbedo.x, fbAlbedo.y, fbAlbedo.z, scwAcc) : make_float4(albedoAcc.x, albedoAcc.y, albedoAcc.z, scwAcc);
                        rec[3] = make_float4(boundsHits, candidates, 0, 0);
                        pix = -1;
                    }
                    if (pix >= 0 && chained) {
                        float *oc = C.outColor, *on = C.outNormal, *oa = C.outAlbedo, *os = C.outScw;
                        if (grouped) { const ChainBatch cb = C.chainBatches[batch]; oc = cb.outColor; on = cb.outNormal; oa = cb.outAlbedo; os = cb.outScw; }
                        reinterpret_cast<float4*>(oc)[pix] = make_float4(colorAcc.x, colorAcc.y, colorAcc.z, (float)sampleCount);
// ... 176 lines not shown
                        const float* ia = (newBatch == 0u ? C.inAlbedo : C.outAlbedo) + 3 * (size_t)pix;
                        last = coherent_load4(ic);
                        normalAcc = coherent_load3(in_);
                        albedoAcc = coherent_load3(ia);
                        scwAcc = coherent_load((newBatch == 0u ? C.inScw : C.outScw) + pix);
                    } else if (!C.probeOnly) {
                        last = reinterpret_cast<const float4*>(C.inColor)[pix];
                        normalAcc = v3(C.inNormal[3 * (size_t)pix], C.inNormal[3 * (size_t)pix + 1], C.inNormal[3 * (size_t)pix + 2]);
                        albedoAcc = v3(C.inAlbedo[3 * (size_t)pix], C.inAlbedo[3 * (size_t)pix + 1], C.inAlbedo[3 * (size_t)pix + 2]);
                        scwAcc = C.inScw[pix];
                    }
                    colorAcc = v3(last.x, last.y, last.z);
                    sampleCount = (int)last.w;
                    }
                    const float scwIn = scwAcc;
                    const int countIn = sampleCount;

                    rng.begin_pixel(NoiseSite{&A, (unsigned)cx, (unsigned)cy}, (unsigned)pix, chained ? C.chainBatches[newBatch].seed : C.seed);

                    const float w = scwIn / (float)countIn;
                    if (w == 0) {
                        nsamp = C.sampleCountMin;
                    } else {
                        const RtowFloat2* const fed = chained ? C.chainBatches[newBatch].extrema : C.extremaIn;
                        const float ex = fed ? fed->x : C.extremaX, ey = fed ? fed->y : C.extremaY;
                        const float nw = um_saturate((w - ex) / (ey - ex));
                        const float lo = (float)C.sampleCountMin, hi = (float)C.sampleCountMax;
                        nsamp = (unsigned)__builtin_rintf(lo + nw * (hi - lo));
                    }
                    if (C.probeOnly) nsamp = (unsigned)C.probeOnly;
                    scw0 = w;
                    smp = 0;
                    if (PER_SAMPLE) {
                        smp = unitGroup * kSampleGroup;
                        nsamp = nsamp < smp + kSampleGroup ? nsamp : smp + kSampleGroup;
                        if (nsamp < smp) nsamp = smp;
                        colorAcc = v3(0, 0, 0); normalAcc = v3(0, 0, 0); albedoAcc = v3(0, 0, 0);
                        sampleCount = 0;
                        scwAcc = 0;
                    }
                    rayCount = 0; boundsHits = 0; candidates = 0;
                    if (WIDE || LONG_LISTS) pcand = C.pixelCandidates ? reinterpret_cast<const uint4*>(C.pixelCandidates)[pix] : make_uint4(WIDE ? 0xffffffffu : kNoPrimaryList, 0u, 0u, 0u);
                    else { const uint2 pc = C.pixelCandidates ? C.pixelCandidates[2 * (size_t)pix] : make_uint2(kNoPrimaryList, 0u); pcand = make_uint4(pc.x, pc.y, 0u, 0u); }
                }
                if (st == ST_REGEN) {
                    const SampleKernelArgs& VA = COLD_VIEW ? cold_args(A) : A;
                    const RtowView& VW = LDS_VIEW ? *reinterpret_cast<const RtowView*>(ldsConst) : VA.view;
                    const float frameX = LDS_VIEW ? ldsConst[29] : VA.sizeX, frameY = LDS_VIEW ? ldsConst[30] : VA.sizeY;
                    const V3 viewRight = PINHOLE ? v3(0, 0, 0) : v3(VW.right), viewUp = PINHOLE ? v3(0, 0, 0) : v3(VW.up);
                    const V3 viewLLC = v3(VW.lowerLeftCorner), viewH = v3(VW.horizontal), viewV = v3(VW.vertical);
                    const float lensRadius = PINHOLE ? 0.0f : VW.lensRadius;
                    float jx = 0.5f, jy = 0.5f;
                    const NoiseSite at{&A, (unsigned)cx, (unsigned)cy};
                    if (PER_SAMPLE) rng.begin_sample(at, (unsigned)pix, smp);
                    if (A.subPixelJitter) rng.next2(at, jx, jy);
                    const float u = ((float)cx + jx) / frameX;
                    const float v = ((float)cy + jy) / frameY;
                    float rdx = 0, rdy = 0;
                    if (lensRadius != 0) {
                        float dx, dy;
                        rng.in_unit_disk(at, dx, dy);
                        rdx = lensRadius * dx;
                        rdy = lensRadius * dy;
                    }
                    const V3 offset = v3(viewRight.x * rdx + viewUp.x * rdy, viewRight.y * rdx + viewUp.y * rdy, viewRight.z * rdx + viewUp.z * rdy);
                    ro = add(v3(VW.origin), offset);
                    rd = normalize(v3(viewLLC.x - offset.x + u * viewH.x + v * viewV.x,
                                      viewLLC.y - offset.y + u * viewH.y + v * viewV.y,
                                      viewLLC.z - offset.z + u * viewH.z + v * viewV.z));
                    rtime = rng.next(at);
                    if (HAS_MOTION) { if (L.commonTimeRange) rtime = um_max(0.0f, um_min(1.0f, (rtime - L.commonT0) / (L.commonT1 - L.commonT0))); }

                    depth = 0;
                    hist.clear();
                    sampleNormal = v3(0, 0, 0);
                    firstNs = -1;
                    randomEventsLocal = 0;
                    curVol = -1;
                    pendRE = 0;
                    startRay();
                    if (WIDE ? !(pcand.x == 0xffffffffu && pcand.y != 0xffffffffu) : pcand.x != kNoPrimaryList) {
                        const f2 invx = {inv.x, inv.x}, invy = {inv.y, inv.y}, invz = {inv.z, inv.z};
                        const f2 ox = {ro.x, ro.x}, oy = {ro.y, ro.y}, oz = {ro.z, ro.z};
                        cur = -1;
                        for (int k = 0; k < 4; k++) {
                            const unsigned node = WIDE ? (k == 0 ? pcand.x : k == 1 ? pcand.y : k == 2 ? pcand.z : pcand.w)
                                                       : ((k < 2 ? pcand.x >> (16 * k) : pcand.y >> (16 * (k - 2))) & 0xffffu);
                            if (node == (WIDE ? 0xffffffffu : 0xffffu)) break;
                            float4 q0, q1, q2;
                            int c0, c1;
                            load_node<ALL_LDS, SPLIT_NODES>(sc, L, (int)node, q0, q1, q2, c0, c1);
                            const f2 tlx = (f2{q0.x, q0.y} - ox) * invx, thx = (f2{q1.z, q1.w} - ox) * invx;
                            const f2 tly = (f2{q0.z, q0.w} - oy) * invy, thy = (f2{q2.x, q2.y} - oy) * invy;
                            const f2 tlz = (f2{q1.x, q1.y} - oz) * invz, thz = (f2{q2.z, q2.w} - oz) * invz;
                            const float tmin0 = vmax3(vmin(tlx.x, thx.x), vmin(tly.x, thy.x), vmax(vmin(tlz.x, thz.x), 0.0f));
                            const float tfar0 = vmin3(vmax(tlx.x, thx.x), vmax(tly.x, thy.x), vmax(tlz.x, thz.x));
                            const float tmin1 = vmax3(vmin(tlx.y, thx.y), vmin(tly.y, thy.y), vmax(vmin(tlz.y, thz.y), 0.0f));
                            const float tfar1 = vmin3(vmax(tlx.y, thx.y), vmax(tly.y, thy.y), vmax(tlz.y, thz.y));
                            const bool leaf0 = c0 < 0 && tmin0 < tfar0;
                            const bool leaf1 = c1 < 0 && tmin1 < tfar1 && twoChildren;
                            if (FULL_DIAG && !refDiag) boundsHits += (leaf0 ? 1.0f : 0.0f) + (leaf1 ? 1.0f : 0.0f);
                            cand[nc * BT] = (Code)~c0;
                            nc += leaf0 ? 1 : 0;
                            cand[nc * BT] = (Code)~c1;
                            nc += leaf1 ? 1 : 0;
                        }
                        if (LONG_LISTS) { if ((pcand.z & 0xffffu) != 0xffffu) cur = -6; }
                        if (nc == 0 && cur == -1) classify(); else st = ST_TEST;
                    }
                }
            }
        }
        if (due(st == ST_TRAV, ST_TRAV, A.tune[1])) {
            ran = true;
            STAGE_MARK(1);
            if (st == ST_TRAV) {
                const f2 invx = {inv.x, inv.x}, invy = {inv.y, inv.y}, invz = {inv.z, inv.z};
                const f2 ox = {ro.x, ro.x}, oy = {ro.y, ro.y}, oz = {ro.z, ro.z};
                int budget = A.travSlice;
                const float bestPrune = best * 1.000244140625f;
                const int candExit = VOLUMES ? kCandCapacity - 2 : (A.tune[6] < kCandCapacity - 1 ? A.tune[6] : kCandCapacity - 1) - 1;
                while (budget > 0 && cur >= 0 && nc <= candExit) {
                    budget--;
                    STAT_ADD(3, (threadIdx.x & 63) == __builtin_ctzll(__ballot(1)) ? 1 : 0);
                    STAT_LANES(4);
                    float4 q0, q1, q2;
                    int c0, c1;
                    load_node<ALL_LDS, SPLIT_NODES>(sc, L, cur, q0, q1, q2, c0, c1);
                    const int spm1 = sp > 0 ? sp - 1 : 0;
                    const int popped = (int)stack[spm1 * BT];
                    const f2 tlx = (f2{q0.x, q0.y} - ox) * invx, thx = (f2{q1.z, q1.w} - ox) * invx;
                    const f2 tly = (f2{q0.z, q0.w} - oy) * invy, thy = (f2{q2.x, q2.y} - oy) * invy;
                    const f2 tlz = (f2{q1.x, q1.y} - oz) * invz, thz = (f2{q2.z, q2.w} - oz) * invz;
                    const float tmin0 = vmax3(vmin(tlx.x, thx.x), vmin(tly.x, thy.x), vmax(vmin(tlz.x, thz.x), 0.0f));
                    const float tfar0 = vmin3(vmax(tlx.x, thx.x), vmax(tly.x, thy.x), vmax(tlz.x, thz.x));
                    const float tmin1 = vmax3(vmin(tlx.y, thx.y), vmin(tly.y, thy.y), vmax(vmin(tlz.y, thz.y), 0.0f));
                    const float tfar1 = vmin3(vmax(tlx.y, thx.y), vmax(tly.y, thy.y), vmax(tlz.y, thz.y));
                    const bool hit0 = tmin0 <= vmin(tfar0, bestPrune);
                    const bool hit1 = tmin1 <= vmin(tfar1, bestPrune) && twoChildren;
                    const bool leaf0 = c0 < 0 && hit0 && tmin0 < tfar0, leaf1 = c1 < 0 && hit1 && tmin1 < tfar1;
                    if (FULL_DIAG && !refDiag) boundsHits += ((c0 < 0 ? leaf0 : hit0) ? 1.0f : 0.0f) + ((c1 < 0 ? leaf1 : hit1) ? 1.0f : 0.0f);
                    cand[nc * BT] = (Code)~c0;
                    nc += leaf0 ? 1 : 0;
                    cand[nc * BT] = (Code)~c1;
                    nc += leaf1 ? 1 : 0;
                    if (PREFETCH_TRI) {
                        if (leaf0) prefetch_sector(sc.glob, L.triHotOffset + (uint32_t)~c0 * (uint32_t)sizeof(GpuTriHot), ldsDump);
                        if (leaf1) prefetch_sector(sc.glob, L.triHotOffset + (uint32_t)~c1 * (uint32_t)sizeof(GpuTriHot), ldsDump);
                    }
                    const bool in0 = hit0 && c0 >= 0;
                    const bool in1 = hit1 && c1 >= 0;
                    const bool both = in0 && in1;
                    const bool swap = tmin1 < tmin0;
                    if (PREFETCH_FAR) {
                        const uint32_t farNode = (uint32_t)(swap ? c0 : c1);
                        if (both && farNode >= sc.ldsNodeCount) prefetch_sector(sc.glob, L.nodeOffset + farNode * 64u, ldsDump);
                    }
                    stack[sp * BT] = (Code)(swap ? c0 : c1);
                    const int next = both ? (swap ? c1 : c0) : (in0 ? c0 : c1);
                    const bool any = in0 || in1;
                    cur = any ? next : (sp > 0 ? popped : -1);
                    sp = any ? sp + (both ? 1 : 0) : spm1;
                }
                if (cur < 0 || nc > candExit) {
                    if (nc > 0) st = ST_TEST;
                    else classify();
                }
            }
        }
        if (due(st == ST_TEST, ST_TEST, A.tune[2])) {
            ran = true;
            STAGE_MARK(2);
            if (st == ST_TEST) {
                const float a = dot(rd, rd);
                for (;;) {
                if (LONG_LISTS) {
                    if (cur <= -2) {
                        const f2 invx = {inv.x, inv.x}, invy = {inv.y, inv.y}, invz = {inv.z, inv.z};
                        const f2 ox = {ro.x, ro.x}, oy = {ro.y, ro.y}, oz = {ro.z, ro.z};
                        int k = -2 - cur;
                        cur = -1;
                        for (; k < 8; k++) {
                            if (nc > kCandCapacity - 2) { cur = -2 - k; break; }
                            const unsigned word = k < 6 ? pcand.z : pcand.w;
                            const unsigned node = (word >> (16 * (k & 1))) & 0xffffu;
                            if (node == 0xffffu) break;
                            float4 q0, q1, q2;
                            int c0, c1;
                            load_node<ALL_LDS, SPLIT_NODES>(sc, L, (int)node, q0, q1, q2, c0, c1);
                            const f2 tlx = (f2{q0.x, q0.y} - ox) * invx, thx = (f2{q1.z, q1.w} - ox) * invx;
                            const f2 tly = (f2{q0.z, q0.w} - oy) * invy, thy = (f2{q2.x, q2.y} - oy) * invy;
                            const f2 tlz = (f2{q1.x, q1.y} - oz) * invz, thz = (f2{q2.z, q2.w} - oz) * invz;
                            const float tmin0 = vmax3(vmin(tlx.x, thx.x), vmin(tly.x, thy.x), vmax(vmin(tlz.x, thz.x), 0.0f));
                            const float tfar0 = vmin3(vmax(tlx.x, thx.x), vmax(tly.x, thy.x), vmax(tlz.x, thz.x));
                            const float tmin1 = vmax3(vmin(tlx.y, thx.y), vmin(tly.y, thy.y), vmax(vmin(tlz.y, thz.y), 0.0f));
                            const float tfar1 = vmin3(vmax(tlx.y, thx.y), vmax(tly.y, thy.y), vmax(tlz.y, thz.y));
                            const bool leaf0 = c0 < 0 && tmin0 < tfar0;
                            const bool leaf1 = c1 < 0 && tmin1 < tfar1 && twoChildren;
                            if (FULL_DIAG && !refDiag) boundsHits += (leaf0 ? 1.0f : 0.0f) + (leaf1 ? 1.0f : 0.0f);
                            cand[nc * BT] = (Code)~c0;
                            nc += leaf0 ? 1 : 0;
                            cand[nc * BT] = (Code)~c1;
                            nc += leaf1 ? 1 : 0;
                        }
                    }
                }
                if (FULL_DIAG && !refDiag) candidates += (float)nc;
                while (nc > 0) {
                    STAT_ADD(5, (threadIdx.x & 63) == __builtin_ctzll(__ballot(1)) ? 1 : 0);
                    STAT_LANES(6);
                    nc--;
                    const int i = (int)cand[nc * BT];
                    if (VOLUMES) {
                        const unsigned mw = *reinterpret_cast<const unsigned*>(section<ALL_LDS>(sc, L.matIndexOffset) + (uint32_t)i * 4u);
                        const unsigned type = mw >> kPrimTypeShift;
                        float tmin = 0.0f;
                        for (int pass = 0; pass < 2; pass++) {
                            float t; V3 nl; float4 rq;
                            if (!general_hit<ALL_LDS>(sc, L, i, type, ro, rd, rtime, tmin, t, nl, rq)) break;
                            const float dn = dot(normalize(rotate(rq, nl)), rd);
                            const unsigned code = (unsigned)i | (dn < 0 ? 0x40000000u : 0u) | (dn > 0 ? 0x80000000u : 0u);
                            if (nHits < kMaxHits) {
                                hitT[nHits] = t; hitTmin0[nHits] = tmin; hitCode[nHits] = code;
                                nHits++;
                            } else if ((unsigned)(nHits - kMaxHits) < A.hitSpillEntries && A.hitSpill) {
                                hit_set(hitT, hitTmin0, hitCode, hit_spill_of(A), nHits, HitRec{t, tmin, code});
                                nHits++;
                            } else {
                                hitOverflow = true;
                            }
                            if (((mw >> 16) & 3u) != MAT_CLASS_VOLUME || !(type == RTOW_ENTITY_BOX || type == RTOW_ENTITY_SPHERE)) break;
                            tmin = t + 0.001f;
                        }
                    } else if (GENERAL) {
                        const unsigned type = TRIANGLES_ONLY ? (unsigned)RTOW_ENTITY_TRIANGLE : *reinterpret_cast<const unsigned*>(section<ALL_LDS>(sc, L.matIndexOffset) + (uint32_t)i * 4u) >> kPrimTypeShift;
                        float t; V3 nl = v3(0, 0, 0); float4 rq;
                        if (TRI_HOT ? tri_hit_hot<ALL_LDS>(sc, L, i, ro, rd, 0.0f, t, nl.x, nl.y) : general_hit<ALL_LDS, TRIANGLES_ONLY>(sc, L, i, type, ro, rd, rtime, 0.0f, t, nl, rq)) {
                            const unsigned* rank = reinterpret_cast<const unsigned*>(section<ALL_LDS>(sc, L.rankOffset));
                            const bool tie = t == best && prim >= 0;
                            if (TIE_WATCH) {
                                if (tie) {
                                    unsigned* const bits = cold_args(A).tieBits;
                                    if (bits) atomicOr(bits + ((unsigned)pix >> 5), 1u << ((unsigned)pix & 31u));
                                }
                            }
                            const unsigned rankHeld = tie ? rank[prim] : 0u;
                            const bool take = t < best || (tie && rank[i] < rankHeld);
                            if (EXACT_TIES) tieAtBest = tie ? true : (t < best ? false : tieAtBest);
                            best = take ? t : best;
                            prim = take ? i : prim;
                            if (KEEP_NORMAL) { keptNormal.x = take ? nl.x : keptNormal.x; keptNormal.y = take ? nl.y : keptNormal.y; if (!TRI_HOT) keptNormal.z = take ? nl.z : keptNormal.z; }
                        }
                    } else {
                        V3 c; float r, t;
                        sphere_at<ALL_LDS, HAS_MOTION>(sc, L, i, rtime, c, r);
                        if (sphere_hit(sub(ro, c), rd, a, r, t) && t <= best) {
                            const unsigned* rank = reinterpret_cast<const unsigned*>(section<ALL_LDS>(sc, L.rankOffset));
                            if (EXACT_TIES) tieAtBest = !(t < best) && prim >= 0;
                            if (TIE_WATCH) {
                                bool take = t < best;
                                if (!take && prim >= 0) {
                                    take = rank[i] < rank[prim];
                                    unsigned* const bits = cold_args(A).tieBits;
                                    if (bits) atomicOr(bits + ((unsigned)pix >> 5), 1u << ((unsigned)pix & 31u));
                                }
                                if (take) { best = t; prim = i; }
                            } else if (t < best || (prim >= 0 && rank[i] < rank[prim])) { best = t; prim = i; }
                        }
                    }
                }
                if (!LONG_LISTS || cur > -2) break;
                }
                if (cur >= 0) st = ST_TRAV;
                else classify();
            }
        }
        if (due(st == ST_HIT, ST_HIT, A.tune[3])) {
            ran = true;
            STAGE_MARK(3);
// ... 305 lines not shown
                                chosen = exitHitIndex;
                                break;
                            }
                            nHits = 0;
                            break;
                        }
                        chosen = hitIndex;
                        break;
                    }
                    if (insideHit) { prim = -1; st = ST_HIT; }
                    else if (chosen >= 0 && chosen < nHits) { best = distAt(chosen); hitTmin = tminAt(chosen); prim = (int)(codeAt(chosen) & kHitPrimMask); st = ST_HIT; }
                    else st = ST_SKY;
                };
                const HitSpill spill = hit_spill_of(A);
                if (nHits > kMaxHits) sort_hit_list_spilled(hitT, hitTmin0, hitCode, spill, nHits, reinterpret_cast<const unsigned*>(section<ALL_LDS>(sc, L.rankOffset)));
                else if (nHits > 1) sort_hit_list(hitT, hitTmin0, hitCode, nHits, reinterpret_cast<const unsigned*>(section<ALL_LDS>(sc, L.rankOffset)));
                volumeLogic([&](int i) { return hit_get(hitT, hitTmin0, hitCode, spill, i).t; }, [&](int i) { return hit_get(hitT, hitTmin0, hitCode, spill, i).code; },
                            [&](int i) { return hit_get(hitT, hitTmin0, hitCode, spill, i).tmin0; });
            }
        }
        if (due(st == ST_SKY, ST_SKY, A.tune[4])) {
            ran = true;
            STAGE_MARK(4);
            STAT_ADD(15, 1);
            if (st == ST_SKY) {
                DBG_TRACE(2, 0xffff, 0.0f);
                V3 sky = v3(0, 0, 0);
                const SampleKernelArgs& EA = COLD_VIEW ? cold_args(A) : A;
                const RtowEnvironment& ENV = LDS_VIEW ? *reinterpret_cast<const RtowEnvironment*>(ldsConst + 22) : EA.environment;
                if (ENV.skyType == RTOW_SKY_GRADIENT) {
                    const float s = 0.5f * (rd.y + 1);
                    const V3 b = v3(ENV.skyBottomColor), tp = v3(ENV.skyTopColor);
                    sky = v3(b.x + s * (tp.x - b.x), b.y + s * (tp.y - b.y), b.z + s * (tp.z - b.z));
                } else if (ENV.skyType == RTOW_SKY_CUBEMAP) {
                    sky = cubemap_sample(cold_args(A).cubemap, rd);
                }
                if (VOLUMES) { randomEventsLocal += pendRE * inv_pow2(depth); pendRE = 0; }
                if (firstNs < 0) sampleNormal = neg(rd);

                V3 col = sky;
                for (int i = depth - 1; i >= 0; i--) {
                    const unsigned code = hist.get(i, histRows);
                    const uint8_t* mp = section<ALL_LDS>(sc, L.materialOffset) + (code & 0x7fffu) * 64u;
                    const float4 m0 = *reinterpret_cast<const float4*>(mp);
                    const float2 m1 = *reinterpret_cast<const float2*>(mp + 16);
                    const bool white = (code & 0x8000u) != 0;
                    if (TEXTURED) {
                        const V3 att = white ? v3(1, 1, 1) : v3(texHist[i * 6 + 0], texHist[i * 6 + 1], texHist[i * 6 + 2]);
                        col = v3(col.x * att.x + texHist[i * 6 + 3], col.y * att.y + texHist[i * 6 + 4], col.z * att.z + texHist[i * 6 + 5]);
                        continue;
                    }
                    const unsigned wmask = (unsigned)((int)(code << 16) >> 31);
                    auto pick = [&](float albedo) { return __uint_as_float((__float_as_uint(albedo) & ~wmask) | (0x3f800000u & wmask)); };
                    const V3 att = v3(pick(m0.x), pick(m0.y), pick(m0.z));
                    col = v3(col.x * att.x + m0.w, col.y * att.y + m1.x, col.z * att.z + m1.y);
                }
                endSample(true, col, sky);
            }
        }
        STAGE_MARK(7);
        if (ran) {
            force = -1;
        } else {
            int top = 0;
            force = -1;
            for (int k = ST_REGEN; k < ST_COUNT; k++) {
                const int n = (int)__popcll(__ballot(st == k));
                if (n > top) { top = n; force = k; }
            }
            if (top == 0) {
                if (!chained || __ballot(st == ST_IDLE) == 0ull) break;
                __builtin_amdgcn_s_sleep(64);
                if (st == ST_IDLE) st = ST_REGEN;
                force = ST_REGEN;
            }
        }
    }
}

template <bool ALL_LDS, int KIND, int HW, int DIAG, int NOISE, bool PER_SAMPLE, int GEO = 0>
hipError_t launchVariant(const SampleKernelArgs& args, int numBlocks, hipStream_t stream)
{
    auto k = sample_batch_kernel<ALL_LDS, KIND, HW, DIAG, NOISE, PER_SAMPLE, GEO>;
    const size_t ldsBytes = (size_t)args.ldsFrontBytes + (size_t)kQueueBytes + args.ldsSceneBytes;
    if (args.ldsStackRows < 1u || ldsBytes > (size_t)kLdsBytesMax) return hipErrorInvalidValue;
    if (HW == 32 && args.traceDepth > kHistoryInRegisters) {
        const uint32_t rows = (uint32_t)(args.traceDepth - kHistoryInRegisters);
        if ((args.ldsHistRows > 0u && args.ldsHistOffset == 0u) || (args.ldsHistRows < rows && (ALL_LDS || !args.histSpill || args.histSpillRows < rows - args.ldsHistRows))) return hipErrorInvalidValue;
    }
    hipError_t e = hipFuncSetAttribute(reinterpret_cast<const void*>(k), hipFuncAttributeMaxDynamicSharedMemorySize, (int)ldsBytes);
    if (e != hipSuccess) return e;
    hipLaunchKernelGGL(k, dim3(numBlocks), dim3(geo_block_threads(GEO)), ldsBytes, stream, args);
    return hipGetLastError();
}

template <int KIND>
constexpr bool kTiesWithShortHistory = true;

template <bool ALL_LDS, int KIND, int GEO>
hipError_t launchByDiagGeo(const SampleKernelArgs& args, int numBlocks, hipStream_t stream)
{
    constexpr bool TIES = (KIND & kExactTiesBit) != 0;
    constexpr bool WIDE = (GEO & kGeoWide) != 0;
    const bool fullDiag = args.diagnostics && args.diagnosticsStride >= 16;
    const int hw = historyWords(args.noiseColor, args.unitRecords != nullptr, WIDE, TIES, fullDiag, args.traceDepth);
    constexpr bool HAS_HURRY_TWIN = RTOW_URGENT_LANES && !WIDE && !TIES && (KIND & 7) == SCENE_KIND_SPHERES;
    const bool hurry = ((uint32_t)args.tune[7] >> 8) != 0u;
    if (hurry && !hurryTwin(KIND & 7, TIES, WIDE, args.noiseColor, args.unitRecords != nullptr, fullDiag, args.refTree != nullptr, args.traceDepth)) return hipErrorInvalidValue;
    if (args.noiseColor == RTOW_NOISE_BLUE) return launchVariant<ALL_LDS, KIND, 32, 2, RTOW_NOISE_BLUE, false, GEO>(args, numBlocks, stream);
    if (args.noiseColor == RTOW_NOISE_SPATIOTEMPORAL_BLUE) return launchVariant<ALL_LDS, KIND, 32, 2, RTOW_NOISE_SPATIOTEMPORAL_BLUE, false, GEO>(args, numBlocks, stream);
    if (args.unitRecords) {
        if constexpr (!TIES && !WIDE) if (hw == 4) return launchVariant<ALL_LDS, KIND, 4, 0, RTOW_NOISE_WHITE, true, GEO>(args, numBlocks, stream);
        return launchVariant<ALL_LDS, KIND, 32, 2, RTOW_NOISE_WHITE, true, GEO>(args, numBlocks, stream);
    }
    constexpr bool HAS_PINHOLE_TWIN = RTOW_PINHOLE && !ALL_LDS && !WIDE && (KIND & 7) == SCENE_KIND_SPHERES;
    const RtowView& vw = args.view;
    const bool pinhole = vw.lensRadius == 0.0f && vw.origin.x != 0.0f && vw.origin.y != 0.0f && vw.origin.z != 0.0f &&
                         vw.lowerLeftCorner.x != 0.0f && vw.lowerLeftCorner.y != 0.0f && vw.lowerLeftCorner.z != 0.0f;
    if constexpr (HAS_PINHOLE_TWIN) {
        if (pinhole && hw == 4) return launchVariant<ALL_LDS, KIND, 4, 0, RTOW_NOISE_WHITE, false, GEO | kGeoPinhole>(args, numBlocks, stream);
        if (pinhole && hw == 8) return launchVariant<ALL_LDS, KIND, 8, 0, RTOW_NOISE_WHITE, false, GEO | kGeoPinhole>(args, numBlocks, stream);
    }
    if (hw == 4) return launchVariant<ALL_LDS, KIND, 4, 0, RTOW_NOISE_WHITE, false, GEO>(args, numBlocks, stream);
    if constexpr (WIDE) {
        if constexpr (TIES) { if (hw == 8) return launchVariant<ALL_LDS, KIND, 8, 0, RTOW_NOISE_WHITE, false, GEO>(args, numBlocks, stream); }
    } else {
        if (hw == 8) return launchVariant<ALL_LDS, KIND, 8, 0, RTOW_NOISE_WHITE, false, GEO>(args, numBlocks, stream);
        if constexpr (HAS_HURRY_TWIN) { if (hurry && !fullDiag) return launchVariant<ALL_LDS, KIND, 32, 0, RTOW_NOISE_WHITE, false, GEO | kGeoHurry>(args, numBlocks, stream); }
        if (!fullDiag) return launchVariant<ALL_LDS, KIND, 32, 0, RTOW_NOISE_WHITE, false, GEO>(args, numBlocks, stream);
    }
    if (args.refTree) return launchVariant<ALL_LDS, KIND, 32, 2, RTOW_NOISE_WHITE, false, GEO>(args, numBlocks, stream);
    if constexpr (HAS_HURRY_TWIN) { if (hurry) return launchVariant<ALL_LDS, KIND, 32, 1, RTOW_NOISE_WHITE, false, GEO | kGeoHurry>(args, numBlocks, stream); }
    return launchVariant<ALL_LDS, KIND, 32, 1, RTOW_NOISE_WHITE, false, GEO>(args, numBlocks, stream);
}

template <int KIND>
constexpr bool kind_has_wide_codes() { return true; }

template <bool ALL_LDS, int KIND>
hipError_t launchByDiag(const SampleKernelArgs& args, int numBlocks, hipStream_t stream)
{
    if constexpr (!ALL_LDS && kind_has_wide_codes<KIND>()) {
        if (args.wideCodes) return launchByDiagGeo<false, KIND, kGeoWide>(args, numBlocks, stream);
    }
    if (args.wideCodes) return hipErrorInvalidValue;
    if (args.blockThreads != kBlockThreads) return hipErrorInvalidValue;
    return launchByDiagGeo<ALL_LDS, KIND, 0>(args, numBlocks, stream);
}

}

#define RTOW_DEFINE_KIND_LAUNCHER(NAME, KIND)                                                                                         \
    hipError_t NAME(const SampleKernelArgs& args, int numBlocks, hipStream_t stream, bool allLds)                                    \
    {                                                                                                                                 \
        return allLds ? launchByDiag<true, KIND>(args, numBlocks, stream) : launchByDiag<false, KIND>(args, numBlocks, stream);     \
    }

}
```

Measured before the change: 9543.

## Add sign-ordered BVH node image in LDS for sphere traversal slab tests

```diff
diff --git a/include/rtow.h b/include/rtow.h
--- a/include/rtow.h
+++ b/include/rtow.h
@@ -208,6 +208,7 @@
     RTOW_CONTEXT_NO_CHUNK_ORDER = 1u << 4,
     RTOW_CONTEXT_FORCE_WIDE_CODES = 1u << 5,
     RTOW_CONTEXT_NO_CHAIN_FUSION = 1u << 7,
+    RTOW_CONTEXT_NODE_IMAGE_64 = 1u << 8,
     RTOW_CONTEXT_NO_THRESHOLD_TUNING = 1u << 6
 } RtowContextFlags;
 
diff --git a/raytracing-in-one-weekend_amd/abi.py b/raytracing-in-one-weekend_amd/abi.py
--- a/raytracing-in-one-weekend_amd/abi.py
+++ b/raytracing-in-one-weekend_amd/abi.py
@@ -125,6 +125,7 @@
 
 
 CONTEXT_EXACT_TIES_ALWAYS, CONTEXT_EXACT_TIES_NEVER, CONTEXT_REFERENCE_DIAGNOSTICS, CONTEXT_NO_CAMERA_RAY_LISTS, CONTEXT_NO_CHUNK_ORDER, CONTEXT_FORCE_WIDE_CODES, CONTEXT_NO_THRESHOLD_TUNING, CONTEXT_NO_CHAIN_FUSION = 1, 2, 4, 8, 16, 32, 64, 128
+CONTEXT_NODE_IMAGE_64 = 256
 GATHER_COLOR, GATHER_NORMAL, GATHER_ALBEDO, GATHER_SAMPLE_COUNT_WEIGHT, GATHER_ALL, GATHER_NO_BATCH_WAIT, GATHER_LOOPBACK = 1, 2, 4, 8, 15, 16, 32
 
 
diff --git a/raytracing-in-one-weekend_amd/csrc/rtow_api.hip b/raytracing-in-one-weekend_amd/csrc/rtow_api.hip
--- a/raytracing-in-one-weekend_amd/csrc/rtow_api.hip
+++ b/raytracing-in-one-weekend_amd/csrc/rtow_api.hip
@@ -150,6 +150,7 @@
     a.layout = ctx->scene.layout;
     a.ldsSceneBytes = ctx->ldsSceneBytes;
     a.ldsNodeCount = ctx->ldsNodeCount;
+    a.ldsNodeImageBytes = ctx->ldsPlan.nodeImageBytes;
     a.ldsStackRows = ctx->ldsPlan.stackRows; a.ldsHistOffset = 0u; a.ldsFrontBytes = ctx->ldsPlan.frontBytes;
     a.workCounter = ctx->dWorkCounter;
     a.cancelFlag = useCancelFlag ? ctx->hCancel : nullptr;
@@ -212,7 +213,7 @@
     if (hw != 32 || a.traceDepth <= kHistoryInRegisters) return RTOW_SUCCESS;
     const LdsPlan plan = planLds(ctx->wideCodes, ctx->scene.layout, (uint32_t)(a.traceDepth - kHistoryInRegisters), ctx->ldsSceneBudget);
     a.ldsStackRows = plan.stackRows; a.ldsHistOffset = plan.histOffset; a.ldsFrontBytes = plan.frontBytes; a.ldsHistRows = plan.histRows;
-    a.ldsSceneBytes = plan.sceneBytes; a.ldsNodeCount = plan.nodeCount;
+    a.ldsSceneBytes = plan.sceneBytes; a.ldsNodeCount = plan.nodeCount; a.ldsNodeImageBytes = plan.nodeImageBytes;
     if (plan.histSpillRows) {
         const size_t stride = (size_t)ctx->cuCount * (size_t)kBlockThreads, need = (size_t)plan.histSpillRows * stride * sizeof(unsigned short);
         if (need > ctx->histSpillBytes) HIP_TRY(ctx, hipDeviceSynchronize(), RTOW_ERROR_LAUNCH_FAILURE);
@@ -225,7 +226,7 @@
 void setSchedulerValues(const RtowContext_t* ctx, const RtowSampleParams* p, SampleKernelArgs& a)
 {
     for (int i = 0; i < 8; i++) a.tune[i] = ctx->tune[i] < 1 ? 1 : ctx->tune[i];
-    a.travSlice = ctx->tune[8] < 1 ? 1 : ctx->tune[8];
+    a.travSlice = travSliceOf(ctx->tune[8]);
     const unsigned unitSamples = p->rngPolicy != RTOW_RNG_REFERENCE ? kSampleGroup : (a.sampleCountMax > a.sampleCountMin ? a.sampleCountMax : a.sampleCountMin);
     const int pixelGate = ctx->pixelGateOverride ? ctx->pixelGateOverride : (unitSamples <= 64u ? 4 : RTOW_PIXEL_GATE);
     const bool records16 = a.diagnostics && a.diagnosticsStride >= 16;
@@ -1033,7 +1034,10 @@
     }
     std::lock_guard<std::mutex> sceneLock(ctx->sceneMu);
     ctx->scene = std::move(compiled);
-    ctx->ldsPlan = planLds(wide, ctx->scene.layout, 0u, ctx->ldsSceneBudget);
+    const SceneLayout& sl = ctx->scene.layout;
+    const bool nodeImage = !wide && sl.sceneKind == SCENE_KIND_SPHERES && !(ctx->flags & RTOW_CONTEXT_NODE_IMAGE_64) &&
+                           node_planes_ordered(reinterpret_cast<const GpuNode*>(ctx->scene.blob.data() + sl.nodeOffset), sl.nodeCount, sl.sphereCount > 1u);
+    ctx->ldsPlan = planLds(wide, sl, 0u, ctx->ldsSceneBudget, nodeImage);
     ctx->ldsSceneBytes = ctx->ldsPlan.sceneBytes;
     ctx->ldsNodeCount = ctx->ldsPlan.nodeCount;
     ctx->haveScene = true;
@@ -1051,9 +1055,9 @@
                 ctx->tunedCandidate = e.winner;
                 ctx->tunedScene = ctx->sceneSerial;
             }
-    logf(ctx, 4, "scene", "%d entities, %u BVH nodes, depth %u, %u bytes (%u in LDS)%s", ctx->scene.entityCount, ctx->scene.layout.nodeCount,
+    logf(ctx, 4, "scene", "%d entities, %u BVH nodes, depth %u, %u bytes (%u in LDS)%s%s", ctx->scene.entityCount, ctx->scene.layout.nodeCount,
          ctx->scene.layout.bvhDepth, ctx->scene.layout.totalBytes, ctx->ldsSceneBytes,
-         ctx->scene.layout.exactTies ? ", exact-tie kernels" : "");
+         ctx->scene.layout.exactTies ? ", exact-tie kernels" : "", ctx->ldsPlan.nodeImageBytes ? ", 80-byte node image" : "");
     return RTOW_SUCCESS;
 }
 
@@ -1141,7 +1145,7 @@
     info->materialCount = ctx->scene.materialCount;
     info->bvhNodeCount = (int32_t)ctx->scene.layout.nodeCount;
     info->bvhDepth = (int32_t)ctx->scene.layout.bvhDepth;
-    info->ldsBytesScene = (int32_t)ctx->ldsSceneBytes;
+    info->ldsBytesScene = (int32_t)(ctx->ldsSceneBytes + ctx->ldsPlan.nodeImageBytes);
     info->sceneInLds = ctx->ldsSceneBytes == ctx->scene.layout.totalBytes ? 1 : 0;
     info->sceneBytesDevice = ctx->scene.layout.totalBytes;
     info->hitSpillBytes = (uint64_t)ctx->hitSpillEntries * (uint64_t)ctx->cuCount * (uint64_t)kBlockThreads * sizeof(uint4);
diff --git a/raytracing-in-one-weekend_amd/csrc/rtow_kernels.h b/raytracing-in-one-weekend_amd/csrc/rtow_kernels.h
--- a/raytracing-in-one-weekend_amd/csrc/rtow_kernels.h
+++ b/raytracing-in-one-weekend_amd/csrc/rtow_kernels.h
@@ -19,6 +19,28 @@
 constexpr int kCandCapacity = 8;
 constexpr int kQueueBytes = 384;
 constexpr int kHistoryInRegisters = 8;
+
+constexpr uint32_t kNodeImageBytes = 80u;
+constexpr uint32_t kNodeImageFlag = 1u << 16;
+inline int32_t travSliceOf(int32_t requested) { return requested < 1 ? 1 : requested >= (int32_t)kNodeImageFlag ? (int32_t)kNodeImageFlag - 1 : requested; }
+inline int32_t travSliceForImage(int32_t slice, bool imageGranted) { return travSliceOf(slice & (int32_t)(kNodeImageFlag - 1u)) | (imageGranted ? (int32_t)kNodeImageFlag : 0); }
+__host__ __device__ inline void node_image(const uint32_t n[16], uint32_t o[20])
+{
+    for (int axis = 0; axis < 3; axis++) {
+        uint32_t* b = o + 6 * axis;
+        b[0] = n[2 * axis]; b[1] = n[2 * axis + 1];
+        b[2] = n[6 + 2 * axis]; b[3] = n[6 + 2 * axis + 1];
+        b[4] = n[2 * axis]; b[5] = n[2 * axis + 1];
+    }
+    o[18] = n[12]; o[19] = n[13];
+}
+inline bool node_planes_ordered(const GpuNode* nodes, uint32_t nodeCount, bool twoChildren)
+{
+    for (uint32_t i = 0; i < nodeCount; i++)
+        for (int c = 0; c < (twoChildren ? 2 : 1); c++)
+            if (!(nodes[i].lox[c] <= nodes[i].hix[c] && nodes[i].loy[c] <= nodes[i].hiy[c] && nodes[i].loz[c] <= nodes[i].hiz[c])) return false;
+    return true;
+}
 
 struct LdsPlan {
     uint32_t stackRows;
@@ -29,8 +51,9 @@
     uint32_t sceneBytes;
     uint32_t nodeCount;
     bool allLds;
-};
-inline LdsPlan planLds(bool wide, const SceneLayout& L, uint32_t histRowsNeeded, uint32_t budgetOverride)
+    uint32_t nodeImageBytes;
+};
+inline LdsPlan planLds(bool wide, const SceneLayout& L, uint32_t histRowsNeeded, uint32_t budgetOverride, bool nodeImage = false)
 {
     LdsPlan p{};
     const uint32_t codeBytes = wide ? 4u : 2u, rowBytes = (uint32_t)kBlockThreads * 2u;
@@ -51,6 +74,9 @@
     if (budget > sceneBudget) budget = sceneBudget;
     if (whole) {
         p.sceneBytes = L.totalBytes; p.nodeCount = L.nodeCount; p.allLds = true;
+        const uint64_t growth = (uint64_t)L.nodeCount * (kNodeImageBytes - (uint32_t)sizeof(GpuNode));
+        if (nodeImage && L.nodeOffset == 0u && (uint64_t)L.totalBytes + growth <= sceneBudget && (uint64_t)L.totalBytes + growth + (uint64_t)histRowsNeeded * rowBytes <= (uint64_t)room)
+            p.nodeImageBytes = (uint32_t)growth;
     } else {
         uint32_t nodes = budget / (uint32_t)sizeof(GpuNode);
         if (nodes > L.nodeCount) nodes = L.nodeCount;
@@ -236,6 +262,7 @@
 
     int32_t tune[8];
     int32_t travSlice;
+    uint32_t ldsNodeImageBytes;
 };
 
 struct KernelInfo {
diff --git a/raytracing-in-one-weekend_amd/csrc/rtow_sample_kernel.hip.h b/raytracing-in-one-weekend_amd/csrc/rtow_sample_kernel.hip.h
--- a/raytracing-in-one-weekend_amd/csrc/rtow_sample_kernel.hip.h
+++ b/raytracing-in-one-weekend_amd/csrc/rtow_sample_kernel.hip.h
@@ -25,6 +25,9 @@
 #endif
 #ifndef RTOW_PINHOLE
 #define RTOW_PINHOLE 1
+#endif
+#ifndef RTOW_SIGNED_WALK
+#define RTOW_SIGNED_WALK 1
 #endif
 #ifndef RTOW_TIE_WATCH
 #define RTOW_TIE_WATCH 1
@@ -628,6 +631,34 @@
     return make_float2(bh, cc);
 }
 
+template <bool ALL_LDS, int KIND, int HW, int DIAG, int NOISE, bool PER_SAMPLE, int GEO>
+constexpr bool signed_walk_variant() { return RTOW_SIGNED_WALK && ALL_LDS && KIND == SCENE_KIND_SPHERES && (HW == 4 || HW == 8) && DIAG == 0 && NOISE == RTOW_NOISE_WHITE && !PER_SAMPLE && GEO == 0; }
+__device__ __forceinline__ uint32_t near_plane_offset(float invAxis) { return (__float_as_uint(invAxis) >> 28) & 8u; }
+__device__ __forceinline__ bool finite_value(float x) { return __builtin_amdgcn_classf(x, 0x1f8); }
+__device__ __forceinline__ bool finite_nonzero(float x) { return __builtin_amdgcn_classf(x, 0x198); }
+__device__ __forceinline__ f2 axis_distances(f2 planes, f2 oi)
+{
+    f2 d, t;
+    asm("v_pk_add_f32 %0, %1, %2 op_sel_hi:[1,0] neg_lo:[0,1] neg_hi:[0,1]" : "=v"(d) : "v"(planes), "v"(oi));
+    asm("v_pk_mul_f32 %0, %1, %2 op_sel:[0,1] op_sel_hi:[1,1]" : "=v"(t) : "v"(d), "v"(oi));
+    return t;
+}
+__device__ __forceinline__ void load_node_image(const uint8_t* image, int idx, uint32_t offx, uint32_t offy, uint32_t offz, float4& px, float4& py, float4& pz, int& c0, int& c1)
+{
+#if defined(__HIP_DEVICE_COMPILE__)
+    typedef __attribute__((address_space(3))) const uint8_t* LdsBytes;
+    typedef float4 PlaneQuad __attribute__((aligned(8)));
+    LdsBytes b = (LdsBytes)image + __umul24((uint32_t)idx, kNodeImageBytes);
+    px = *(__attribute__((address_space(3))) const PlaneQuad*)(b + offx);
+    py = *(__attribute__((address_space(3))) const PlaneQuad*)(b + 24u + offy);
+    pz = *(__attribute__((address_space(3))) const PlaneQuad*)(b + 48u + offz);
+    const int2 c = *(__attribute__((address_space(3))) const int2*)(b + 72u);
+    c0 = c.x; c1 = c.y;
+#else
+    (void)image; (void)idx; (void)offx; (void)offy; (void)offz; px = py = pz = make_float4(0, 0, 0, 0); c0 = c1 = -1;
+#endif
+}
+
 constexpr int kGeoWide = 4;
 constexpr int kGeoPinhole = 8;
 constexpr int kGeoHurry = 16;
@@ -647,6 +678,7 @@
     constexpr bool LDS_VIEW = (RTOW_LDS_VIEW & (ALL_LDS ? 1 : 2)) != 0;
     constexpr bool COLD_VIEW __attribute__((unused)) = RTOW_COLD_VIEW && !ALL_LDS && !LDS_VIEW;
     constexpr bool SPLIT_NODES = !ALL_LDS && !WIDE;
+    constexpr bool SIGNED_WALK = signed_walk_variant<ALL_LDS, KIND, HW, DIAG, NOISE, PER_SAMPLE, GEO>();
     using Code = typename std::conditional<WIDE, unsigned, unsigned short>::type;
     const uint32_t ldsFront = A.ldsFrontBytes;
 
@@ -668,7 +700,20 @@
         ldsConst[tid] = *reinterpret_cast<const float*>(ka + from);
     }
 #endif
-    {
+    uint32_t imageGrowth = 0;
+    if (SIGNED_WALK && (A.travSlice & (int)kNodeImageFlag) != 0) {
+        const uint4* src = reinterpret_cast<const uint4*>(A.sceneBlob);
+        const uint32_t nodes = A.layout.nodeCount, n16 = A.ldsSceneBytes >> 4;
+        imageGrowth = nodes * (kNodeImageBytes - (uint32_t)sizeof(GpuNode));
+        uint4* img = reinterpret_cast<uint4*>(ldsScene);
+        for (uint32_t i = (uint32_t)tid; i < nodes; i += BT) {
+            uint4 in[4] = {src[4u * i], src[4u * i + 1u], src[4u * i + 2u], src[4u * i + 3u]}, out[5];
+            node_image(reinterpret_cast<const uint32_t*>(in), reinterpret_cast<uint32_t*>(out));
+            for (int k = 0; k < 5; k++) img[5u * i + (uint32_t)k] = out[k];
+        }
+        uint4* dst = reinterpret_cast<uint4*>(ldsScene + imageGrowth);
+        for (uint32_t i = 4u * nodes + (uint32_t)tid; i < n16; i += BT) dst[i] = src[i];
+    } else {
         const uint4* src = reinterpret_cast<const uint4*>(A.sceneBlob);
         uint4* dst = reinterpret_cast<uint4*>(ldsScene);
         const uint32_t n16 = A.ldsSceneBytes >> 4;
@@ -677,7 +722,7 @@
     __syncthreads();
 
     SceneRefs sc;
-    sc.lds = ldsScene;
+    sc.lds = ldsScene + imageGrowth;
     sc.glob = A.sceneBlob;
     sc.ldsNodeCount = A.ldsNodeCount;
     const SceneLayout L = A.layout;
@@ -776,6 +821,44 @@
         }
         smp++;
         st = ST_REGEN;
+    };
+    auto signOrderedWave = [&]() -> bool {
+        if (!SIGNED_WALK || (A.travSlice & (int)kNodeImageFlag) == 0) return false;
+        const bool ok = finite_value(ro.x) && finite_value(ro.y) && finite_value(ro.z) && finite_nonzero(inv.x) && finite_nonzero(inv.y) && finite_nonzero(inv.z);
+        return __ballot(!ok) == 0ull;
+    };
+    auto loadNode = [&](int idx, float4& q0, float4& q1, float4& q2, int& c0, int& c1) {
+        if (SIGNED_WALK && (A.travSlice & (int)kNodeImageFlag) != 0) {
+            float4 px, py, pz;
+            load_node_image(ldsScene, idx, 0u, 0u, 0u, px, py, pz, c0, c1);
+            q0 = make_float4(px.x, px.y, py.x, py.y); q1 = make_float4(pz.x, pz.y, px.z, px.w); q2 = make_float4(py.z, py.w, pz.z, pz.w);
+        } else {
+            load_node<ALL_LDS, SPLIT_NODES>(sc, L, idx, q0, q1, q2, c0, c1);
+        }
+    };
+    auto nodeSlabs = [&](int idx, bool ordered, float& tmin0, float& tfar0, float& tmin1, float& tfar1, int& c0, int& c1) {
+        const f2 invx = {inv.x, inv.x}, invy = {inv.y, inv.y}, invz = {inv.z, inv.z};
+        const f2 ox = {ro.x, ro.x}, oy = {ro.y, ro.y}, oz = {ro.z, ro.z};
+        if (SIGNED_WALK && ordered) {
+            float4 px, py, pz;
+            load_node_image(ldsScene, idx, near_plane_offset(inv.x), near_plane_offset(inv.y), near_plane_offset(inv.z), px, py, pz, c0, c1);
+            const f2 oix = {ro.x, inv.x}, oiy = {ro.y, inv.y}, oiz = {ro.z, inv.z};
+            const f2 tnx = axis_distances(f2{px.x, px.y}, oix), tfx = axis_distances(f2{px.z, px.w}, oix);
+            const f2 tny = axis_distances(f2{py.x, py.y}, oiy), tfy = axis_distances(f2{py.z, py.w}, oiy);
+            const f2 tnz = axis_distances(f2{pz.x, pz.y}, oiz), tfz = axis_distances(f2{pz.z, pz.w}, oiz);
+            tmin0 = vmax3(tnx.x, tny.x, vmax(tnz.x, 0.0f)); tfar0 = vmin3(tfx.x, tfy.x, tfz.x);
+            tmin1 = vmax3(tnx.y, tny.y, vmax(tnz.y, 0.0f)); tfar1 = vmin3(tfx.y, tfy.y, tfz.y);
+        } else {
+            float4 q0, q1, q2;
+            loadNode(idx, q0, q1, q2, c0, c1);
+            const f2 tlx = (f2{q0.x, q0.y} - ox) * invx, thx = (f2{q1.z, q1.w} - ox) * invx;
+            const f2 tly = (f2{q0.z, q0.w} - oy) * invy, thy = (f2{q2.x, q2.y} - oy) * invy;
+            const f2 tlz = (f2{q1.x, q1.y} - oz) * invz, thz = (f2{q2.z, q2.w} - oz) * invz;
+            tmin0 = vmax3(vmin(tlx.x, thx.x), vmin(tly.x, thy.x), vmax(vmin(tlz.x, thz.x), 0.0f));
+            tfar0 = vmin3(vmax(tlx.x, thx.x), vmax(tly.x, thy.x), vmax(tlz.x, thz.x));
+            tmin1 = vmax3(vmin(tlx.y, thx.y), vmin(tly.y, thy.y), vmax(vmin(tlz.y, thz.y), 0.0f));
+            tfar1 = vmin3(vmax(tlx.y, thx.y), vmax(tly.y, thy.y), vmax(tlz.y, thz.y));
+        }
     };
     auto startRay = [&]() {
         inv = v3(RTOW_RCP_NAN_TO_INF(rd.x), RTOW_RCP_NAN_TO_INF(rd.y), RTOW_RCP_NAN_TO_INF(rd.z));
@@ -1118,21 +1201,27 @@
                     if (WIDE ? !(pcand.x == 0xffffffffu && pcand.y != 0xffffffffu) : pcand.x != kNoPrimaryList) {
                         const f2 invx = {inv.x, inv.x}, invy = {inv.y, inv.y}, invz = {inv.z, inv.z};
                         const f2 ox = {ro.x, ro.x}, oy = {ro.y, ro.y}, oz = {ro.z, ro.z};
+                        const bool ordered = signOrderedWave();
                         cur = -1;
                         for (int k = 0; k < 4; k++) {
                             const unsigned node = WIDE ? (k == 0 ? pcand.x : k == 1 ? pcand.y : k == 2 ? pcand.z : pcand.w)
                                                        : ((k < 2 ? pcand.x >> (16 * k) : pcand.y >> (16 * (k - 2))) & 0xffffu);
                             if (node == (WIDE ? 0xffffffffu : 0xffffu)) break;
-                            float4 q0, q1, q2;
+                            float tmin0, tfar0, tmin1, tfar1;
                             int c0, c1;
-                            load_node<ALL_LDS, SPLIT_NODES>(sc, L, (int)node, q0, q1, q2, c0, c1);
-                            const f2 tlx = (f2{q0.x, q0.y} - ox) * invx, thx = (f2{q1.z, q1.w} - ox) * invx;
-                            const f2 tly = (f2{q0.z, q0.w} - oy) * invy, thy = (f2{q2.x, q2.y} - oy) * invy;
-                            const f2 tlz = (f2{q1.x, q1.y} - oz) * invz, thz = (f2{q2.z, q2.w} - oz) * invz;
-                            const float tmin0 = vmax3(vmin(tlx.x, thx.x), vmin(tly.x, thy.x), vmax(vmin(tlz.x, thz.x), 0.0f));
-                            const float tfar0 = vmin3(vmax(tlx.x, thx.x), vmax(tly.x, thy.x), vmax(tlz.x, thz.x));
-                            const float tmin1 = vmax3(vmin(tlx.y, thx.y), vmin(tly.y, thy.y), vmax(vmin(tlz.y, thz.y), 0.0f));
-                            const float tfar1 = vmin3(vmax(tlx.y, thx.y), vmax(tly.y, thy.y), vmax(tlz.y, thz.y));
+                            if constexpr (SIGNED_WALK) {
+                                nodeSlabs((int)node, ordered, tmin0, tfar0, tmin1, tfar1, c0, c1);
+                            } else {
+                                float4 q0, q1, q2;
+                                load_node<ALL_LDS, SPLIT_NODES>(sc, L, (int)node, q0, q1, q2, c0, c1);
+                                const f2 tlx = (f2{q0.x, q0.y} - ox) * invx, thx = (f2{q1.z, q1.w} - ox) * invx;
+                                const f2 tly = (f2{q0.z, q0.w} - oy) * invy, thy = (f2{q2.x, q2.y} - oy) * invy;
+                                const f2 tlz = (f2{q1.x, q1.y} - oz) * invz, thz = (f2{q2.z, q2.w} - oz) * invz;
+                                tmin0 = vmax3(vmin(tlx.x, thx.x), vmin(tly.x, thy.x), vmax(vmin(tlz.x, thz.x), 0.0f));
+                                tfar0 = vmin3(vmax(tlx.x, thx.x), vmax(tly.x, thy.x), vmax(tlz.x, thz.x));
+                                tmin1 = vmax3(vmin(tlx.y, thx.y), vmin(tly.y, thy.y), vmax(vmin(tlz.y, thz.y), 0.0f));
+                                tfar1 = vmin3(vmax(tlx.y, thx.y), vmax(tly.y, thy.y), vmax(tlz.y, thz.y));
+                            }
                             const bool leaf0 = c0 < 0 && tmin0 < tfar0;
                             const bool leaf1 = c1 < 0 && tmin1 < tfar1 && twoChildren;
                             if (FULL_DIAG && !refDiag) boundsHits += (leaf0 ? 1.0f : 0.0f) + (leaf1 ? 1.0f : 0.0f);
@@ -1153,50 +1242,117 @@
             if (st == ST_TRAV) {
                 const f2 invx = {inv.x, inv.x}, invy = {inv.y, inv.y}, invz = {inv.z, inv.z};
                 const f2 ox = {ro.x, ro.x}, oy = {ro.y, ro.y}, oz = {ro.z, ro.z};
-                int budget = A.travSlice;
+                int budget = SIGNED_WALK ? A.travSlice & (int)(kNodeImageFlag - 1u) : A.travSlice;
                 const float bestPrune = best * 1.000244140625f;
                 const int candExit = VOLUMES ? kCandCapacity - 2 : (A.tune[6] < kCandCapacity - 1 ? A.tune[6] : kCandCapacity - 1) - 1;
-                while (budget > 0 && cur >= 0 && nc <= candExit) {
-                    budget--;
-                    STAT_ADD(3, (threadIdx.x & 63) == __builtin_ctzll(__ballot(1)) ? 1 : 0);
-                    STAT_LANES(4);
-                    float4 q0, q1, q2;
-                    int c0, c1;
-                    load_node<ALL_LDS, SPLIT_NODES>(sc, L, cur, q0, q1, q2, c0, c1);
-                    const int spm1 = sp > 0 ? sp - 1 : 0;
-                    const int popped = (int)stack[spm1 * BT];
-                    const f2 tlx = (f2{q0.x, q0.y} - ox) * invx, thx = (f2{q1.z, q1.w} - ox) * invx;
-                    const f2 tly = (f2{q0.z, q0.w} - oy) * invy, thy = (f2{q2.x, q2.y} - oy) * invy;
-                    const f2 tlz = (f2{q1.x, q1.y} - oz) * invz, thz = (f2{q2.z, q2.w} - oz) * invz;
-                    const float tmin0 = vmax3(vmin(tlx.x, thx.x), vmin(tly.x, thy.x), vmax(vmin(tlz.x, thz.x), 0.0f));
-                    const float tfar0 = vmin3(vmax(tlx.x, thx.x), vmax(tly.x, thy.x), vmax(tlz.x, thz.x));
-                    const float tmin1 = vmax3(vmin(tlx.y, thx.y), vmin(tly.y, thy.y), vmax(vmin(tlz.y, thz.y), 0.0f));
-                    const float tfar1 = vmin3(vmax(tlx.y, thx.y), vmax(tly.y, thy.y), vmax(tlz.y, thz.y));
-                    const bool hit0 = tmin0 <= vmin(tfar0, bestPrune);
-                    const bool hit1 = tmin1 <= vmin(tfar1, bestPrune) && twoChildren;
-                    const bool leaf0 = c0 < 0 && hit0 && tmin0 < tfar0, leaf1 = c1 < 0 && hit1 && tmin1 < tfar1;
-                    if (FULL_DIAG && !refDiag) boundsHits += ((c0 < 0 ? leaf0 : hit0) ? 1.0f : 0.0f) + ((c1 < 0 ? leaf1 : hit1) ? 1.0f : 0.0f);
-                    cand[nc * BT] = (Code)~c0;
-                    nc += leaf0 ? 1 : 0;
-                    cand[nc * BT] = (Code)~c1;
-                    nc += leaf1 ? 1 : 0;
-                    if (PREFETCH_TRI) {
-                        if (leaf0) prefetch_sector(sc.glob, L.triHotOffset + (uint32_t)~c0 * (uint32_t)sizeof(GpuTriHot), ldsDump);
-                        if (leaf1) prefetch_sector(sc.glob, L.triHotOffset + (uint32_t)~c1 * (uint32_t)sizeof(GpuTriHot), ldsDump);
-                    }
-                    const bool in0 = hit0 && c0 >= 0;
-                    const bool in1 = hit1 && c1 >= 0;
-                    const bool both = in0 && in1;
-                    const bool swap = tmin1 < tmin0;
-                    if (PREFETCH_FAR) {
-                        const uint32_t farNode = (uint32_t)(swap ? c0 : c1);
-                        if (both && farNode >= sc.ldsNodeCount) prefetch_sector(sc.glob, L.nodeOffset + farNode * 64u, ldsDump);
-                    }
-                    stack[sp * BT] = (Code)(swap ? c0 : c1);
-                    const int next = both ? (swap ? c1 : c0) : (in0 ? c0 : c1);
-                    const bool any = in0 || in1;
-                    cur = any ? next : (sp > 0 ? popped : -1);
-                    sp = any ? sp + (both ? 1 : 0) : spm1;
+                if constexpr (SIGNED_WALK) {
+                    auto finishVisit = [&](float tmin0, float tfar0, float tmin1, float tfar1, int c0, int c1, int popped, int spm1) {
+                        const bool hit0 = tmin0 <= vmin(tfar0, bestPrune);
+                        const bool hit1 = tmin1 <= vmin(tfar1, bestPrune) && twoChildren;
+                        const bool leaf0 = c0 < 0 && hit0 && tmin0 < tfar0, leaf1 = c1 < 0 && hit1 && tmin1 < tfar1;
+                        if (FULL_DIAG && !refDiag) boundsHits += ((c0 < 0 ? leaf0 : hit0) ? 1.0f : 0.0f) + ((c1 < 0 ? leaf1 : hit1) ? 1.0f : 0.0f);
+                        cand[nc * BT] = (Code)~c0;
+                        nc += leaf0 ? 1 : 0;
+                        cand[nc * BT] = (Code)~c1;
+                        nc += leaf1 ? 1 : 0;
+                        if (PREFETCH_TRI) {
+                            if (leaf0) prefetch_sector(sc.glob, L.triHotOffset + (uint32_t)~c0 * (uint32_t)sizeof(GpuTriHot), ldsDump);
+                            if (leaf1) prefetch_sector(sc.glob, L.triHotOffset + (uint32_t)~c1 * (uint32_t)sizeof(GpuTriHot), ldsDump);
+                        }
+                        const bool in0 = hit0 && c0 >= 0;
+                        const bool in1 = hit1 && c1 >= 0;
+                        const bool both = in0 && in1;
+                        const bool swap = tmin1 < tmin0;
+                        if (PREFETCH_FAR) {
+                            const uint32_t farNode = (uint32_t)(swap ? c0 : c1);
+                            if (both && farNode >= sc.ldsNodeCount) prefetch_sector(sc.glob, L.nodeOffset + farNode * 64u, ldsDump);
+                        }
+                        stack[sp * BT] = (Code)(swap ? c0 : c1);
+                        const int next = both ? (swap ? c1 : c0) : (in0 ? c0 : c1);
+                        const bool any = in0 || in1;
+                        cur = any ? next : (sp > 0 ? popped : -1);
+                        sp = any ? sp + (both ? 1 : 0) : spm1;
+                    };
+                    if (signOrderedWave()) {
+                        const uint32_t offx = near_plane_offset(inv.x), offy = near_plane_offset(inv.y), offz = near_plane_offset(inv.z);
+                        const f2 oix = {ro.x, inv.x}, oiy = {ro.y, inv.y}, oiz = {ro.z, inv.z};
+                        while (budget > 0 && cur >= 0 && nc <= candExit) {
+                            budget--;
+                            STAT_ADD(3, (threadIdx.x & 63) == __builtin_ctzll(__ballot(1)) ? 1 : 0);
+                            STAT_LANES(4);
+                            float4 px, py, pz;
+                            int c0, c1;
+                            load_node_image(ldsScene, cur, offx, offy, offz, px, py, pz, c0, c1);
+                            const int spm1 = sp > 0 ? sp - 1 : 0;
+                            const int popped = (int)stack[spm1 * BT];
+                            const f2 tnx = axis_distances(f2{px.x, px.y}, oix), tfx = axis_distances(f2{px.z, px.w}, oix);
+                            const f2 tny = axis_distances(f2{py.x, py.y}, oiy), tfy = axis_distances(f2{py.z, py.w}, oiy);
+                            const f2 tnz = axis_distances(f2{pz.x, pz.y}, oiz), tfz = axis_distances(f2{pz.z, pz.w}, oiz);
+                            finishVisit(vmax3(tnx.x, tny.x, vmax(tnz.x, 0.0f)), vmin3(tfx.x, tfy.x, tfz.x), vmax3(tnx.y, tny.y, vmax(tnz.y, 0.0f)), vmin3(tfx.y, tfy.y, tfz.y), c0, c1, popped, spm1);
+                        }
+                    } else {
+                        while (budget > 0 && cur >= 0 && nc <= candExit) {
+                            budget--;
+                            STAT_ADD(3, (threadIdx.x & 63) == __builtin_ctzll(__ballot(1)) ? 1 : 0);
+                            STAT_LANES(4);
+                            float4 q0, q1, q2;
+                            int c0, c1;
+                            loadNode(cur, q0, q1, q2, c0, c1);
+                            const int spm1 = sp > 0 ? sp - 1 : 0;
+                            const int popped = (int)stack[spm1 * BT];
+                            const f2 tlx = (f2{q0.x, q0.y} - ox) * invx, thx = (f2{q1.z, q1.w} - ox) * invx;
+                            const f2 tly = (f2{q0.z, q0.w} - oy) * invy, thy = (f2{q2.x, q2.y} - oy) * invy;
+                            const f2 tlz = (f2{q1.x, q1.y} - oz) * invz, thz = (f2{q2.z, q2.w} - oz) * invz;
+                            const float tmin0 = vmax3(vmin(tlx.x, thx.x), vmin(tly.x, thy.x), vmax(vmin(tlz.x, thz.x), 0.0f));
+                            const float tfar0 = vmin3(vmax(tlx.x, thx.x), vmax(tly.x, thy.x), vmax(tlz.x, thz.x));
+                            const float tmin1 = vmax3(vmin(tlx.y, thx.y), vmin(tly.y, thy.y), vmax(vmin(tlz.y, thz.y), 0.0f));
+                            const float tfar1 = vmin3(vmax(tlx.y, thx.y), vmax(tly.y, thy.y), vmax(tlz.y, thz.y));
+                            finishVisit(tmin0, tfar0, tmin1, tfar1, c0, c1, popped, spm1);
+                        }
+                    }
+                } else {
+                    while (budget > 0 && cur >= 0 && nc <= candExit) {
+                        budget--;
+                        STAT_ADD(3, (threadIdx.x & 63) == __builtin_ctzll(__ballot(1)) ? 1 : 0);
+                        STAT_LANES(4);
+                        float4 q0, q1, q2;
+                        int c0, c1;
+                        load_node<ALL_LDS, SPLIT_NODES>(sc, L, cur, q0, q1, q2, c0, c1);
+                        const int spm1 = sp > 0 ? sp - 1 : 0;
+                        const int popped = (int)stack[spm1 * BT];
+                        const f2 tlx = (f2{q0.x, q0.y} - ox) * invx, thx = (f2{q1.z, q1.w} - ox) * invx;
+                        const f2 tly = (f2{q0.z, q0.w} - oy) * invy, thy = (f2{q2.x, q2.y} - oy) * invy;
+                        const f2 tlz = (f2{q1.x, q1.y} - oz) * invz, thz = (f2{q2.z, q2.w} - oz) * invz;
+                        const float tmin0 = vmax3(vmin(tlx.x, thx.x), vmin(tly.x, thy.x), vmax(vmin(tlz.x, thz.x), 0.0f));
+                        const float tfar0 = vmin3(vmax(tlx.x, thx.x), vmax(tly.x, thy.x), vmax(tlz.x, thz.x));
+                        const float tmin1 = vmax3(vmin(tlx.y, thx.y), vmin(tly.y, thy.y), vmax(vmin(tlz.y, thz.y), 0.0f));
+                        const float tfar1 = vmin3(vmax(tlx.y, thx.y), vmax(tly.y, thy.y), vmax(tlz.y, thz.y));
+                        const bool hit0 = tmin0 <= vmin(tfar0, bestPrune);
+                        const bool hit1 = tmin1 <= vmin(tfar1, bestPrune) && twoChildren;
+                        const bool leaf0 = c0 < 0 && hit0 && tmin0 < tfar0, leaf1 = c1 < 0 && hit1 && tmin1 < tfar1;
+                        if (FULL_DIAG && !refDiag) boundsHits += ((c0 < 0 ? leaf0 : hit0) ? 1.0f : 0.0f) + ((c1 < 0 ? leaf1 : hit1) ? 1.0f : 0.0f);
+                        cand[nc * BT] = (Code)~c0;
+                        nc += leaf0 ? 1 : 0;
+                        cand[nc * BT] = (Code)~c1;
+                        nc += leaf1 ? 1 : 0;
+                        if (PREFETCH_TRI) {
+                            if (leaf0) prefetch_sector(sc.glob, L.triHotOffset + (uint32_t)~c0 * (uint32_t)sizeof(GpuTriHot), ldsDump);
+                            if (leaf1) prefetch_sector(sc.glob, L.triHotOffset + (uint32_t)~c1 * (uint32_t)sizeof(GpuTriHot), ldsDump);
+                        }
+                        const bool in0 = hit0 && c0 >= 0;
+                        const bool in1 = hit1 && c1 >= 0;
+                        const bool both = in0 && in1;
+                        const bool swap = tmin1 < tmin0;
+                        if (PREFETCH_FAR) {
+                            const uint32_t farNode = (uint32_t)(swap ? c0 : c1);
+                            if (both && farNode >= sc.ldsNodeCount) prefetch_sector(sc.glob, L.nodeOffset + farNode * 64u, ldsDump);
+                        }
+                        stack[sp * BT] = (Code)(swap ? c0 : c1);
+                        const int next = both ? (swap ? c1 : c0) : (in0 ? c0 : c1);
+                        const bool any = in0 || in1;
+                        cur = any ? next : (sp > 0 ? popped : -1);
+                        sp = any ? sp + (both ? 1 : 0) : spm1;
+                    }
                 }
                 if (cur < 0 || nc > candExit) {
                     if (nc > 0) st = ST_TEST;
@@ -1214,6 +1370,7 @@
                     if (cur <= -2) {
                         const f2 invx = {inv.x, inv.x}, invy = {inv.y, inv.y}, invz = {inv.z, inv.z};
                         const f2 ox = {ro.x, ro.x}, oy = {ro.y, ro.y}, oz = {ro.z, ro.z};
+                        const bool ordered = signOrderedWave();
                         int k = -2 - cur;
                         cur = -1;
                         for (; k < 8; k++) {
@@ -1221,16 +1378,21 @@
                             const unsigned word = k < 6 ? pcand.z : pcand.w;
                             const unsigned node = (word >> (16 * (k & 1))) & 0xffffu;
                             if (node == 0xffffu) break;
-                            float4 q0, q1, q2;
+                            float tmin0, tfar0, tmin1, tfar1;
                             int c0, c1;
-                            load_node<ALL_LDS, SPLIT_NODES>(sc, L, (int)node, q0, q1, q2, c0, c1);
-                            const f2 tlx = (f2{q0.x, q0.y} - ox) * invx, thx = (f2{q1.z, q1.w} - ox) * invx;
-                            const f2 tly = (f2{q0.z, q0.w} - oy) * invy, thy = (f2{q2.x, q2.y} - oy) * invy;
-                            const f2 tlz = (f2{q1.x, q1.y} - oz) * invz, thz = (f2{q2.z, q2.w} - oz) * invz;
-                            const float tmin0 = vmax3(vmin(tlx.x, thx.x), vmin(tly.x, thy.x), vmax(vmin(tlz.x, thz.x), 0.0f));
-                            const float tfar0 = vmin3(vmax(tlx.x, thx.x), vmax(tly.x, thy.x), vmax(tlz.x, thz.x));
-                            const float tmin1 = vmax3(vmin(tlx.y, thx.y), vmin(tly.y, thy.y), vmax(vmin(tlz.y, thz.y), 0.0f));
-                            const float tfar1 = vmin3(vmax(tlx.y, thx.y), vmax(tly.y, thy.y), vmax(tlz.y, thz.y));
+                            if constexpr (SIGNED_WALK) {
+                                nodeSlabs((int)node, ordered, tmin0, tfar0, tmin1, tfar1, c0, c1);
+                            } else {
+                                float4 q0, q1, q2;
+                                load_node<ALL_LDS, SPLIT_NODES>(sc, L, (int)node, q0, q1, q2, c0, c1);
+                                const f2 tlx = (f2{q0.x, q0.y} - ox) * invx, thx = (f2{q1.z, q1.w} - ox) * invx;
+                                const f2 tly = (f2{q0.z, q0.w} - oy) * invy, thy = (f2{q2.x, q2.y} - oy) * invy;
+                                const f2 tlz = (f2{q1.x, q1.y} - oz) * invz, thz = (f2{q2.z, q2.w} - oz) * invz;
+                                tmin0 = vmax3(vmin(tlx.x, thx.x), vmin(tly.x, thy.x), vmax(vmin(tlz.x, thz.x), 0.0f));
+                                tfar0 = vmin3(vmax(tlx.x, thx.x), vmax(tly.x, thy.x), vmax(tlz.x, thz.x));
+                                tmin1 = vmax3(vmin(tlx.y, thx.y), vmin(tly.y, thy.y), vmax(vmin(tlz.y, thz.y), 0.0f));
+                                tfar1 = vmin3(vmax(tlx.y, thx.y), vmax(tly.y, thy.y), vmax(tlz.y, thz.y));
+                            }
                             const bool leaf0 = c0 < 0 && tmin0 < tfar0;
                             const bool leaf1 = c1 < 0 && tmin1 < tfar1 && twoChildren;
                             if (FULL_DIAG && !refDiag) boundsHits += (leaf0 ? 1.0f : 0.0f) + (leaf1 ? 1.0f : 0.0f);
@@ -1702,7 +1864,16 @@
 hipError_t launchVariant(const SampleKernelArgs& args, int numBlocks, hipStream_t stream)
 {
     auto k = sample_batch_kernel<ALL_LDS, KIND, HW, DIAG, NOISE, PER_SAMPLE, GEO>;
-    const size_t ldsBytes = (size_t)args.ldsFrontBytes + (size_t)kQueueBytes + args.ldsSceneBytes;
+    constexpr bool SIGNED_WALK = signed_walk_variant<ALL_LDS, KIND, HW, DIAG, NOISE, PER_SAMPLE, GEO>();
+    const bool imageGranted = SIGNED_WALK && args.ldsNodeImageBytes != 0u && args.ldsNodeImageBytes == args.layout.nodeCount * (kNodeImageBytes - (uint32_t)sizeof(GpuNode));
+    SampleKernelArgs ownSlice;
+    const SampleKernelArgs* launchArgs = &args;
+    if (SIGNED_WALK) {
+        ownSlice = args;
+        ownSlice.travSlice = travSliceForImage(args.travSlice, imageGranted);
+        launchArgs = &ownSlice;
+    }
+    const size_t ldsBytes = (size_t)args.ldsFrontBytes + (size_t)kQueueBytes + args.ldsSceneBytes + (imageGranted ? args.ldsNodeImageBytes : 0u);
     if (args.ldsStackRows < 1u || ldsBytes > (size_t)kLdsBytesMax) return hipErrorInvalidValue;
     if (HW == 32 && args.traceDepth > kHistoryInRegisters) {
         const uint32_t rows = (uint32_t)(args.traceDepth - kHistoryInRegisters);
@@ -1710,7 +1881,7 @@
     }
     hipError_t e = hipFuncSetAttribute(reinterpret_cast<const void*>(k), hipFuncAttributeMaxDynamicSharedMemorySize, (int)ldsBytes);
     if (e != hipSuccess) return e;
-    hipLaunchKernelGGL(k, dim3(numBlocks), dim3(geo_block_threads(GEO)), ldsBytes, stream, args);
+    hipLaunchKernelGGL(k, dim3(numBlocks), dim3(geo_block_threads(GEO)), ldsBytes, stream, *launchArgs);
     return hipGetLastError();
 }
 
```

New measurement: 9748, median of 6. 1.02x the previous value.
